# amankhullar/MMBiDAF

Hardware: NVIDIA B200
Metric: mmbidaf_train_videos_per_s (higher is better)
Workload: dtype bf16 tcgen05 BiDAF + tf32 library GEMMs, fp32 accumulate / soft-max / LSTM

## Files before the change

mmbidaf_b200/csrc/decoder_fused.cu:

```cuda
#include <cooperative_groups.h>
#include <stdlib.h>
#include <type_traits>
#include "common.cuh"
#include "tc_common.cuh"

namespace cg = cooperative_groups;

namespace mmb {
namespace {

constexpr int NT = 512;
constexpr int NW = NT / 32;
constexpr int MAXC = 8;
constexpr int SCR = 2048;
__host__ __device__ constexpr int split4(int n, int parts) { return ((n + parts - 1) / parts + 3) & ~3; }

__device__ __forceinline__ float rcp_ftz(float x) {
  float y;
  asm("rcp.approx.ftz.f32 %0, %1;" : "=f"(y) : "f"(x));
  return y;
}

__device__ __forceinline__ void bulk_reduce_add_f32(float* dst, uint32_t src_smem, uint32_t bytes) {
  asm volatile("cp.reduce.async.bulk.global.shared::cta.bulk_group.add.f32 [%0], [%1], %2;" ::"l"(dst), "r"(src_smem), "r"(bytes)
               : "memory");
}
__device__ __forceinline__ void bulk_commit() { asm volatile("cp.async.bulk.commit_group;" ::: "memory"); }
__device__ __forceinline__ void bulk_wait_all() { asm volatile("cp.async.bulk.wait_group 0;" ::: "memory"); }
__device__ __forceinline__ void red_add_f32_if(float* p, float v, bool on) {
  asm volatile(
      "{\n\t"
      ".reg .pred q;\n\t"
      "setp.ne.b32 q, %2, 0;\n\t"
      "@q red.global.add.f32 [%0], %1;\n\t"
      "}" ::"l"(p), "f"(v), "r"((int)on)
      : "memory");
}

__device__ long long* g_dec_trace = nullptr;
#define DEC_STAMP(i)                                                          \
  do {                                                                        \
    if (g_dec_trace && blockIdx.x == 0 && threadIdx.x == 0) g_dec_trace[i] = clock64(); \
  } while (0)

struct FusedArgs {
  const float *proj_a, *proj_i, *enc_a, *enc_i;
  const float *Wh4t, *bh4;
  const float *v1, *wc1, *v2, *wc2, *v1b, *v2b;
  const float *Wb13t;
  const float *vb1, *vb2, *vb1b, *vb2b;
  const float *Wcatt, *bcat;
  const float *out_wt, *out_b;
  const float *sent, *h, *cell, *cov;
  const uint8_t* mask;
  const long long* target;
  float *probs, *h_out, *cell_out, *att_cov, *cov_out;
  long long* argmax;
  float *nll, *cov_loss;
  float *hw, *alpha, *beta, *ctx12, *pb, *xcat, *gates;
  int B, Lt, D, H, E, M, chunk;
  int stage_off;
};

template <typename ColOf, typename Emit>
__device__ __forceinline__ void block_matvec_t(const float* __restrict__ Wt, const int ldn, const float* __restrict__ bias, const float* x,
                                               const int K, const int n_out, float* scratch, const int scratch_cap, bool quads,
                                               ColOf col_of, Emit emit) {
  const int tid = threadIdx.x;
  if (n_out <= 0) return;
  quads = quads && ((ldn | n_out) & 3) == 0 && (reinterpret_cast<uintptr_t>(Wt) & 15) == 0 && scratch_cap >= 2 * n_out;
  if (quads) {
    const int nq = n_out >> 2;
    const int S = max(1, min(min(NT / nq, scratch_cap / n_out), K));
    const int q = tid % nq, sl = tid / nq;
    float4 acc = make_float4(0.f, 0.f, 0.f, 0.f);
    if (sl < S) {
      const int per = (K + S - 1) / S, k0 = min(K, sl * per), k1 = min(K, k0 + per);
      const float4* w = reinterpret_cast<const float4*>(Wt + (size_t)k0 * ldn + col_of(4 * q));
      const size_t ld4 = (size_t)(ldn >> 2);
      for (int k = k0; k < k1; k += 16) {
        float4 wv[16];
#pragma unroll
        for (int u = 0; u < 16; ++u) wv[u] = k + u < k1 ? __ldcg(w + u * ld4) : make_float4(0.f, 0.f, 0.f, 0.f);
#pragma unroll
        for (int u = 0; u < 16; ++u) {
          const float xv = k + u < k1 ? x[k + u] : 0.f;
          acc.x = fmaf(wv[u].x, xv, acc.x); acc.y = fmaf(wv[u].y, xv, acc.y);
          acc.z = fmaf(wv[u].z, xv, acc.z); acc.w = fmaf(wv[u].w, xv, acc.w);
        }
        w += 16 * ld4;
      }
    }
    __syncthreads();
    if (sl < S) *reinterpret_cast<float4*>(scratch + sl * n_out + 4 * q) = acc;
    __syncthreads();
    if (tid < n_out) {
      float v = 0.f;
      for (int p = 0; p < S; ++p) v += scratch[p * n_out + tid];
      const int c = col_of(tid);
      emit(tid, v + (bias ? __ldg(bias + c) : 0.f));
    }
    return;
  }
  const int S = max(1, min(min(NT / n_out, scratch_cap / n_out), 32));
  const int i = tid % n_out, sl = tid / n_out;
  float acc = 0.f;
  if (sl < S) {
    const int per = (K + S - 1) / S, k0 = min(K, sl * per), k1 = min(K, k0 + per);
    const float* w = Wt + (size_t)k0 * ldn + col_of(i);
    float a0 = 0.f, a1 = 0.f, a2 = 0.f, a3 = 0.f;
    int k = k0;
    for (; k + 16 <= k1; k += 16) {
      float wv[16];
#pragma unroll
      for (int u = 0; u < 16; ++u) wv[u] = __ldcg(w + (size_t)u * ldn);
#pragma unroll
      for (int u = 0; u < 16; u += 4) {
        a0 = fmaf(wv[u], x[k + u], a0); a1 = fmaf(wv[u + 1], x[k + u + 1], a1);
        a2 = fmaf(wv[u + 2], x[k + u + 2], a2); a3 = fmaf(wv[u + 3], x[k + u + 3], a3);
      }
      w += (size_t)16 * ldn;
    }
    if (k + 8 <= k1) {
      float wv[8];
#pragma unroll
      for (int u = 0; u < 8; ++u) wv[u] = __ldcg(w + (size_t)u * ldn);
#pragma unroll
      for (int u = 0; u < 8; u += 4) {
        a0 = fmaf(wv[u], x[k + u], a0); a1 = fmaf(wv[u + 1], x[k + u + 1], a1);
        a2 = fmaf(wv[u + 2], x[k + u + 2], a2); a3 = fmaf(wv[u + 3], x[k + u + 3], a3);
      }
      w += (size_t)8 * ldn;
      k += 8;
    }
    for (; k < k1; ++k) {
      a0 = fmaf(__ldcg(w), x[k], a0);
      w += ldn;
    }
    acc = (a0 + a1) + (a2 + a3);
  }
  __syncthreads();
  if (sl < S && S > 1) scratch[sl * n_out + i] = acc;
  __syncthreads();
  if (tid < n_out) {
    float v = acc;
    for (int q = 1; q < S; ++q) v += scratch[q * n_out + tid];
    const int c = col_of(tid);
    emit(tid, v + (bias ? __ldg(bias + c) : 0.f));
  }
}

__device__ __forceinline__ float block_sum(float v, float* red) {
  const int lane = threadIdx.x & 31, warp = threadIdx.x >> 5;
  v = warp_sum(v);
  __syncthreads();
  if (lane == 0) red[warp] = v;
  __syncthreads();
  float r = lane < NW ? red[lane] : 0.f;
  return warp_sum(r);
}
__device__ __forceinline__ float block_max(float v, float* red) {
  const int lane = threadIdx.x & 31, warp = threadIdx.x >> 5;
  v = warp_max(v);
  __syncthreads();
  if (lane == 0) red[warp] = v;
  __syncthreads();
  float r = lane < NW ? red[lane] : -INFINITY;
  return warp_max(r);
}

struct GreedyArgs {
  const float *emb_text, *h0;
  int steps, T;
};

template <bool kGreedy>
__device__ __forceinline__ void dec_fused_body(const FusedArgs& a, const GreedyArgs& g) {
  cg::cluster_group cluster = cg::this_cluster();
  const int CL = (int)cluster.num_blocks(), R = (int)cluster.block_rank();
  const int b = blockIdx.x / CL;
  const int tid = threadIdx.x, lane = tid & 31, warp = tid >> 5;
  const int D = a.D, H = a.H, E = a.E, M = a.M, Lt = a.Lt, K = D + E + H;

  extern __shared__ __align__(16) float smem[];
  auto up4 = [](int v) { return (v + 3) & ~3; };
  float* s_hw = smem;
  float* s_x = s_hw + up4(4 * D);
  float* s_ctx = s_x + up4(K);
  float* s_pb = s_ctx + up4(2 * D);
  float* s_hn = s_pb + up4(2 * D);
  float* s_part = s_hn + up4(H);
  float* s_ex = s_part + up4(MAXC * (4 + 2 * D));
  float* s_g = s_ex + MAXC * 8;
  float* s_red = s_g + up4(4 * (split4(H, MAXC / 2) + 1));
  float* s_scr = s_red + 32;
  float* s_vec = s_scr + SCR;
  float* s_e = s_vec + up4(4 * D);
  float* s_cov = s_e + up4(2 * a.chunk);
  float* s_cpart = s_cov + up4(a.chunk);

  const int t0 = min(Lt, R * a.chunk), t1 = min(Lt, t0 + a.chunk), n = t1 - t0;
  const bool staged = a.stage_off != 0;
  float* const s_st0 = smem + a.stage_off + 4;
  float* const s_st1 = s_st0 + up4(a.chunk * D);
  const uint32_t bar_proj = tc::smem_u32(smem + a.stage_off), bar_enc = bar_proj + 8;
  const uint32_t stage_bytes = (uint32_t)(n * D) * 4u;
  if (staged && tid == 0) {
    tc::mbar_init(bar_proj, 1);
    tc::mbar_init(bar_enc, 1);
    tc::fence_barrier_init();
    if (n > 0) {
      tc::mbar_expect_tx(bar_proj, 2 * stage_bytes, 1);
      tc::tma_bulk_g2s(tc::smem_u32(s_st0), a.proj_a + ((size_t)b * Lt + t0) * D, stage_bytes, bar_proj, 1);
      tc::tma_bulk_g2s(tc::smem_u32(s_st1), a.proj_i + ((size_t)b * Lt + t0) * D, stage_bytes, bar_proj, 1);
    }
  }
  DEC_STAMP(0);
  const int S = kGreedy ? g.steps : 1;
  float cell_own = 0.f;
  int pick = 0;
  for (int s = 0; s < S; ++s) {
  const uint32_t parity = kGreedy ? (uint32_t)(s & 1) : 0u;
  if constexpr (!kGreedy) {
    for (int i = tid; i < n; i += NT) s_cov[i] = a.cov[(size_t)b * Lt + t0 + i];
    for (int i = tid; i < H; i += NT) s_x[D + E + i] = a.h[(size_t)b * H + i];
    for (int i = tid; i < E; i += NT) s_x[D + i] = a.sent[(size_t)b * E + i];
  } else {
    if (s == 0)
      for (int i = tid; i < n; i += NT) s_cov[i] = 0.f;
    for (int i = tid; i < H; i += NT) s_x[D + E + i] = s == 0 ? g.h0[(size_t)b * H + i] : s_hn[i];
    const float* row = g.emb_text + ((size_t)b * Lt + min(pick, Lt - 1)) * E;
    for (int i = tid; i < E; i += NT) s_x[D + i] = s == 0 ? 0.f : row[i];
  }
  if (!kGreedy || s == 0)
    for (int i = tid; i < D; i += NT) {
      s_vec[i] = a.v1[i];
      s_vec[D + i] = a.wc1[i];
      s_vec[2 * D + i] = a.v2[i];
      s_vec[3 * D + i] = a.wc2[i];
    }
  __syncthreads();

  DEC_STAMP(1);
  {
    const int per = (4 * D + CL - 1) / CL, o0 = R * per, o1 = min(4 * D, o0 + per);
    block_matvec_t(a.Wh4t, 4 * D, a.bh4, s_x + D + E, H, o1 - o0, s_scr, SCR, (o0 & 3) == 0, [&](int i) { return o0 + i; }, [&](int i, float v) {
      const int o = o0 + i;
      for (int r = 0; r < CL; ++r) cluster.map_shared_rank(s_hw, r)[o] = v;
      if constexpr (!kGreedy) a.hw[(size_t)b * 4 * D + o] = v;
    });
  }
  DEC_STAMP(2);
  cluster.sync();
  DEC_STAMP(3);

  {
    const float v1b = a.v1b[0], v2b = a.v2b[0];
    constexpr float K2 = 2.0f * 1.4426950408889634f;
    auto energies = [&](const float* __restrict__ pa0, const float* __restrict__ pi0, auto nj_tag, auto ru_tag) {
      constexpr int NJ = decltype(nj_tag)::value, RU = decltype(ru_tag)::value;
      float va[NJ], ha[NJ], wa[NJ], vi[NJ], hi[NJ], wi[NJ];
#pragma unroll
      for (int j = 0; j < NJ; ++j) {
        const int d = lane + 32 * j;
        const bool in = d < D;
        const int dd = in ? d : 0;
        va[j] = in ? s_vec[dd] : 0.f;
        wa[j] = in ? s_vec[D + dd] * K2 : 0.f;
        ha[j] = in ? s_hw[dd] * K2 : 0.f;
        vi[j] = in ? s_vec[2 * D + dd] : 0.f;
        wi[j] = in ? s_vec[3 * D + dd] * K2 : 0.f;
        hi[j] = in ? s_hw[D + dd] * K2 : 0.f;
      }
      const float* const covp = s_cov;
      for (int i = warp * RU; i < n; i += NW * RU) {
        float s[RU][2];
        float pav[RU][NJ], piv[RU][NJ], cvs[RU];
#pragma unroll
        for (int u = 0; u < RU; ++u) {
          s[u][0] = s[u][1] = 0.f;
          const int r = min(i + u, n - 1);
          const float* pa = pa0 + (size_t)r * D;
          const float* pi = pi0 + (size_t)r * D;
          cvs[u] = covp[r];
#pragma unroll
          for (int j = 0; j < NJ; ++j) {
            const int d = lane + 32 * j;
            pav[u][j] = d < D ? pa[d] : 0.f;
            piv[u][j] = d < D ? pi[d] : 0.f;
          }
        }
#pragma unroll
        for (int u = 0; u < RU; ++u) {
          const float cv = cvs[u];
#pragma unroll
          for (int j = 0; j < NJ; ++j) {
            const float x1 = fmaf(cv, wa[j], fmaf(pav[u][j], K2, ha[j]));
            const float x2 = fmaf(cv, wi[j], fmaf(piv[u][j], K2, hi[j]));
            const float r1 = rcp_ftz(1.0f + tc::fast_exp2(x1)), r2 = rcp_ftz(1.0f + tc::fast_exp2(x2));
            s[u][0] = fmaf(va[j], fmaf(-2.0f, r1, 1.0f), s[u][0]);
            s[u][1] = fmaf(vi[j], fmaf(-2.0f, r2, 1.0f), s[u][1]);
          }
        }
#pragma unroll
        for (int u = 0; u < RU; ++u) {
          const float x1 = warp_sum(s[u][0]), x2 = warp_sum(s[u][1]);
          if (lane == 0 && i + u < n) {
            s_e[i + u] = x1 + v1b;
            s_e[a.chunk + i + u] = x2 + v2b;
          }
        }
      }
    };
    const float* const gpa = a.proj_a + ((size_t)b * Lt + t0) * D;
    const float* const gpi = a.proj_i + ((size_t)b * Lt + t0) * D;
    using N7 = std::integral_constant<int, 7>;
    using N8 = std::integral_constant<int, 8>;
    using R2 = std::integral_constant<int, 2>;
    using R4 = std::integral_constant<int, 4>;
    const bool nj7 = D > 192 && D <= 224;
    if (staged) {
      if (n > 0) tc::mbar_wait(bar_proj, parity);
      if (nj7) energies(s_st0, s_st1, N7{}, R2{});
      else energies(s_st0, s_st1, N8{}, R2{});
    } else {
      if (nj7) energies(gpa, gpi, N7{}, R4{});
      else energies(gpa, gpi, N8{}, R4{});
    }
    __syncthreads();
    if (staged && tid == 0 && n > 0) {
      tc::fence_proxy_async();
      tc::mbar_expect_tx(bar_enc, 2 * stage_bytes, 1);
      tc::tma_bulk_g2s(tc::smem_u32(s_st0), a.enc_a + ((size_t)b * Lt + t0) * D, stage_bytes, bar_enc, 1);
      tc::tma_bulk_g2s(tc::smem_u32(s_st1), a.enc_i + ((size_t)b * Lt + t0) * D, stage_bytes, bar_enc, 1);
    }
    DEC_STAMP(4);
    float m1 = -INFINITY, m2 = -INFINITY;
    for (int i = tid; i < n; i += NT) {
      m1 = fmaxf(m1, s_e[i]);
      m2 = fmaxf(m2, s_e[a.chunk + i]);
    }
    m1 = block_max(m1, s_red);
    m2 = block_max(m2, s_red);
    float l1 = 0.f, l2 = 0.f;
    for (int i = tid; i < n; i += NT) {
      const float p1 = expf(s_e[i] - m1), p2 = expf(s_e[a.chunk + i] - m2);
      s_e[i] = p1;
      s_e[a.chunk + i] = p2;
      l1 += p1;
      l2 += p2;
    }
    l1 = block_sum(l1, s_red);
    l2 = block_sum(l2, s_red);
    __syncthreads();
    DEC_STAMP(5);
    if (staged && n > 0) tc::mbar_wait(bar_enc, parity);
    const float* ea = staged ? s_st0 : a.enc_a + ((size_t)b * Lt + t0) * D;
    const float* ei = staged ? s_st1 : a.enc_i + ((size_t)b * Lt + t0) * D;
    const bool vec4 = (D & 3) == 0;
    const int groups = vec4 ? NT / (D >> 2) : NT / D;
    if (vec4) {
      const int dv4 = D >> 2;
      const int g = tid / dv4, c4 = tid - g * dv4;
      if (g < groups) {
        float4 s1 = make_float4(0.f, 0.f, 0.f, 0.f), s2 = s1;
#pragma unroll 8
        for (int i = g; i < n; i += groups) {
          const float w1 = s_e[i], w2 = s_e[a.chunk + i];
          const float4 x1 = *reinterpret_cast<const float4*>(ea + (size_t)i * D + c4 * 4);
          const float4 x2 = *reinterpret_cast<const float4*>(ei + (size_t)i * D + c4 * 4);
          s1.x = fmaf(w1, x1.x, s1.x); s1.y = fmaf(w1, x1.y, s1.y); s1.z = fmaf(w1, x1.z, s1.z); s1.w = fmaf(w1, x1.w, s1.w);
          s2.x = fmaf(w2, x2.x, s2.x); s2.y = fmaf(w2, x2.y, s2.y); s2.z = fmaf(w2, x2.z, s2.z); s2.w = fmaf(w2, x2.w, s2.w);
        }
        *reinterpret_cast<float4*>(s_cpart + (g * 2 + 0) * D + c4 * 4) = s1;
        *reinterpret_cast<float4*>(s_cpart + (g * 2 + 1) * D + c4 * 4) = s2;
      }
    } else {
      const int g = tid / D, d = tid - g * D;
      if (g < groups) {
        float s1 = 0.f, s2 = 0.f;
        for (int i = g; i < n; i += groups) {
          s1 = fmaf(s_e[i], ea[(size_t)i * D + d], s1);
          s2 = fmaf(s_e[a.chunk + i], ei[(size_t)i * D + d], s2);
        }
        s_cpart[(g * 2 + 0) * D + d] = s1;
        s_cpart[(g * 2 + 1) * D + d] = s2;
      }
    }
    __syncthreads();
    if constexpr (kGreedy) {
      if (staged && tid == 0 && n > 0 && s + 1 < S) {
        tc::fence_proxy_async();
        tc::mbar_expect_tx(bar_proj, 2 * stage_bytes, 1);
        tc::tma_bulk_g2s(tc::smem_u32(s_st0), a.proj_a + ((size_t)b * Lt + t0) * D, stage_bytes, bar_proj, 1);
        tc::tma_bulk_g2s(tc::smem_u32(s_st1), a.proj_i + ((size_t)b * Lt + t0) * D, stage_bytes, bar_proj, 1);
      }
    }
    for (int d = tid; d < 2 * D; d += NT) {
      const int k = d / D, dd = d - k * D;
      float s = 0.f;
      for (int g = 0; g < groups; ++g) s += s_cpart[(g * 2 + k) * D + dd];
      for (int r = 0; r < CL; ++r) cluster.map_shared_rank(s_part, r)[R * (4 + 2 * D) + 4 + d] = s;
    }
    if (tid < CL) {
      float* dst = cluster.map_shared_rank(s_part, tid) + R * (4 + 2 * D);
      dst[0] = m1; dst[1] = l1; dst[2] = m2; dst[3] = l2;
    }
  }
  DEC_STAMP(6);
  cluster.sync();
  DEC_STAMP(7);

  float scale_own[2];
  {
    float* s_w = s_scr;
    if (tid < 2) {
      const int k = tid;
      float m = -INFINITY;
      for (int r = 0; r < CL; ++r)
        if (min(Lt, r * a.chunk) < Lt) m = fmaxf(m, s_part[r * (4 + 2 * D) + 2 * k]);
      float l = 0.f, w[MAXC];
#pragma unroll
      for (int r = 0; r < MAXC; ++r) {
        w[r] = (r < CL && min(Lt, r * a.chunk) < Lt) ? expf(s_part[r * (4 + 2 * D) + 2 * k] - m) : 0.f;
        l = fmaf(w[r], r < CL ? s_part[r * (4 + 2 * D) + 2 * k + 1] : 0.f, l);
      }
      const float inv = 1.f / l;
#pragma unroll
      for (int r = 0; r < MAXC; ++r) s_w[k * MAXC + r] = w[r] * inv;
    }
    __syncthreads();
    scale_own[0] = s_w[R];
    scale_own[1] = s_w[MAXC + R];
    for (int i = tid; i < 2 * D; i += NT) {
      const int k = i / D;
      float sum = 0.f;
      for (int r = 0; r < CL; ++r) sum = fmaf(s_w[k * MAXC + r], s_part[r * (4 + 2 * D) + 4 + i], sum);
      s_ctx[i] = sum;
      if (!kGreedy && R == 0) a.ctx12[((size_t)k * a.B + b) * D + (i - k * D)] = sum;
    }
  }
  __syncthreads();
  DEC_STAMP(8);

  {
    const int per = (2 * D + CL - 1) / CL, o0 = R * per, o1 = min(2 * D, o0 + per);
    for (int k = 0; k < 2; ++k) {
      const int lo = max(o0, k * D), hi = min(o1, (k + 1) * D);
      block_matvec_t(a.Wb13t + (size_t)k * D * D, D, nullptr, s_ctx + k * D, D, hi - lo, s_scr, SCR, ((lo - k * D) & 3) == 0,
                     [&](int i) { return lo - k * D + i; },
                     [&](int i, float v) {
                       const int o = lo + i;
                       for (int r = 0; r < CL; ++r) cluster.map_shared_rank(s_pb, r)[o] = v;
                       if constexpr (!kGreedy) a.pb[((size_t)k * a.B + b) * D + (o - k * D)] = v;
                     });
    }
  }
  DEC_STAMP(9);
  cluster.sync();
  DEC_STAMP(10);
  float beta1, beta2;
  {
    float eb1 = 0.f, eb2 = 0.f;
    for (int d = tid; d < D; d += NT) {
      eb1 = fmaf(a.vb1[d], tanh_fast(s_pb[d] + s_hw[2 * D + d]), eb1);
      eb2 = fmaf(a.vb2[d], tanh_fast(s_pb[D + d] + s_hw[3 * D + d]), eb2);
    }
    eb1 = block_sum(eb1, s_red) + a.vb1b[0];
    eb2 = block_sum(eb2, s_red) + a.vb2b[0];
    const float mb = fmaxf(eb1, eb2);
    const float x1 = expf(eb1 - mb), x2 = expf(eb2 - mb);
    beta1 = x1 / (x1 + x2);
    beta2 = x2 / (x1 + x2);
    for (int d = tid; d < D; d += NT) s_x[d] = s_ctx[d] * beta1 + s_ctx[D + d] * beta2;
    float closs = 0.f;
    for (int i = tid; i < n; i += NT) {
      const int t = t0 + i;
      const float a1 = s_e[i] * scale_own[0], a2 = s_e[a.chunk + i] * scale_own[1];
      if constexpr (!kGreedy) {
        a.alpha[((size_t)b * 2 + 0) * Lt + t] = a1;
        a.alpha[((size_t)b * 2 + 1) * Lt + t] = a2;
      }
      const float att = a1 * beta1 + a2 * beta2;
      if constexpr (kGreedy) {
        const float cnew = s_cov[i] + att;
        s_cov[i] = cnew;
        closs += fminf(att, cnew);
      } else {
        const float cnew = a.cov[(size_t)b * Lt + t] + att;
        a.att_cov[(size_t)b * Lt + t] = att;
        a.cov_out[(size_t)b * Lt + t] = cnew;
        closs += fminf(att, cnew);
      }
    }
    closs = block_sum(closs, s_red);
    if (tid == 0) cluster.map_shared_rank(s_ex, 0)[R * 8 + 0] = closs;
    if (!kGreedy && R == 0 && tid == 0) {
      a.beta[b * 2 + 0] = beta1;
      a.beta[b * 2 + 1] = beta2;
    }
  }
  __syncthreads();
  if (!kGreedy && R == 0)
    for (int i = tid; i < K; i += NT) a.xcat[(size_t)b * K + i] = s_x[i];

  DEC_STAMP(11);
  {
    const int per = split4(H, CL), j0 = R * per, j1 = min(H, j0 + per), nj = max(0, j1 - j0);
    block_matvec_t(a.Wcatt, 4 * H, a.bcat, s_x, K, 4 * nj, s_scr, SCR, ((H | nj) & 3) == 0, [&](int i) { return (i / nj) * H + j0 + (i % nj); },
                   [&](int i, float v) { s_g[(i / nj) * (per + 1) + (i % nj)] = v; });
    __syncthreads();
    if (tid < nj) {
      const int j = j0 + tid;
      const float gi = gate_act(s_g[tid], 1.f), gf = gate_act(s_g[(per + 1) + tid], 1.f), gg = tanh_fast(s_g[2 * (per + 1) + tid]),
                  go = gate_act(s_g[3 * (per + 1) + tid], 1.f);
      const float c = fmaf(gf, kGreedy ? cell_own : a.cell[(size_t)b * H + j], gi * gg);
      const float hn = go * tanh_fast(c);
      if constexpr (kGreedy) {
        cell_own = c;
      } else {
        a.cell_out[(size_t)b * H + j] = c;
        a.h_out[(size_t)b * H + j] = hn;
        float* gs = a.gates + (size_t)b * 4 * H;
        gs[j] = gi; gs[H + j] = gf; gs[2 * H + j] = gg; gs[3 * H + j] = go;
      }
      for (int r = 0; r < CL; ++r) cluster.map_shared_rank(s_hn, r)[j] = hn;
    }
  }
  DEC_STAMP(12);
  cluster.sync();
  DEC_STAMP(13);
  const size_t prow = kGreedy ? (size_t)b * S + s : (size_t)b;
  const int lrow = kGreedy ? s * 2 * a.B + b : b;
  if (R == 0 && tid == 0 && a.cov_loss) {
    float cs = 0.f;
    for (int r = 0; r < CL; ++r) cs += s_ex[r * 8 + 0];
    a.cov_loss[lrow] = cs;
  }

  {
    const int per = (M + CL - 1) / CL, m0 = min(M, R * per), m1 = min(M, m0 + per);
    float* const lg = s_cpart;
    block_matvec_t(a.out_wt, M, a.out_b, s_hn, H, m1 - m0, s_scr, SCR, (m0 & 3) == 0, [&](int i) { return m0 + i; }, [&](int i, float v) { lg[i] = v; });
    __syncthreads();
    for (int m = m0 + tid; m < m1; m += NT)
      if (!a.mask[(size_t)b * M + m]) lg[m - m0] = kNegFill;
    __syncthreads();
    float mx = -INFINITY;
    for (int m = m0 + tid; m < m1; m += NT) mx = fmaxf(mx, lg[m - m0]);
    mx = block_max(mx, s_red);
    float sum = 0.f;
    for (int m = m0 + tid; m < m1; m += NT) sum += expf(lg[m - m0] - mx);
    sum = block_sum(sum, s_red);
    if (tid < CL) {
      float* dst = cluster.map_shared_rank(s_ex, tid) + R * 8;
      dst[1] = mx;
      dst[2] = sum;
    }
    DEC_STAMP(14);
    cluster.sync();
    DEC_STAMP(15);
    float gmx = -INFINITY;
    for (int r = 0; r < CL; ++r)
      if (min(M, r * per) < M) gmx = fmaxf(gmx, s_ex[r * 8 + 1]);
    float gsum = 0.f;
    for (int r = 0; r < CL; ++r)
      if (min(M, r * per) < M) gsum = fmaf(s_ex[r * 8 + 2], expf(s_ex[r * 8 + 1] - gmx), gsum);
    const float inv = 1.f / gsum;
    float best = -INFINITY;
    int best_i = M;
    const int tg = a.target ? (int)a.target[kGreedy ? b * g.T + s : b] : -1;
    for (int m = m0 + tid; m < m1; m += NT) {
      const float p = expf(lg[m - m0] - gmx) * inv;
      a.probs[prow * M + m] = p;
      if (p > best) { best = p; best_i = m; }
      if (m == tg && a.nll) a.nll[lrow] = -logf(p + 1e-12f);
    }
    if (kGreedy || a.argmax) {
      const float bbest = block_max(best, s_red);
      int cand = best == bbest ? best_i : M;
#pragma unroll
      for (int o = 16; o > 0; o >>= 1) cand = min(cand, __shfl_xor_sync(0xffffffffu, cand, o));
      __shared__ int redi[NW];
      __syncthreads();
      if (lane == 0) redi[warp] = cand;
      __syncthreads();
      if (tid == 0) {
        int r = M;
        for (int w = 0; w < NW; ++w) r = min(r, redi[w]);
        for (int q = 0; q < (kGreedy ? CL : 1); ++q) {
          float* dst = cluster.map_shared_rank(s_ex, q) + R * 8;
          dst[3] = bbest;
          dst[4] = __int_as_float(r);
        }
      }
      cluster.sync();
      if (kGreedy || (R == 0 && tid == 0)) {
        float gb = -INFINITY;
        int gi = M;
        for (int r = 0; r < CL; ++r) {
          if (min(M, r * per) >= M) continue;
          const float pb_ = s_ex[r * 8 + 3];
          const int ib = __float_as_int(s_ex[r * 8 + 4]);
          if (pb_ > gb || (pb_ == gb && ib < gi)) { gb = pb_; gi = ib; }
        }
        if constexpr (kGreedy) {
          if (R == 0 && tid == 0) a.argmax[prow] = gi;
          pick = gi;
        } else {
          a.argmax[b] = gi;
        }
      }
    }
  }
  }
  DEC_STAMP(16);
  DEC_STAMP(17);
}

__global__ void __launch_bounds__(NT) dec_step_fused_kernel(const FusedArgs a) { dec_fused_body<false>(a, GreedyArgs{}); }

__global__ void __launch_bounds__(NT) dec_greedy_fused_kernel(const FusedArgs a, const GreedyArgs g) { dec_fused_body<true>(a, g); }

}

struct HeadArgs {
  const float *probs, *d_probs;
  const long long* target;
  const float *g_nll, *g_cov;
  const float* out_w;
  const float *gates, *cell_in, *cell_out;
  const float *d_h_out, *d_cell_out;
  const float* Wcat_ctx;
  const float *d_att_cov, *d_cov_out;
  const float *alpha, *beta, *ctx12, *pb, *hw;
  const float *vb1, *vb2;
  const float *att, *cov_out;
  const float* Wb13;
  float* d_logits;
  float* d_gates;
  float *d_cell, *datt, *dcov_tot, *d_pre_b, *d_ctx12;
  float *vec_acc, *scal_acc;
  int B, Lt, D, H, M, ldd, ldg, chunk;
  int sweeps;
  const float *proj_a, *proj_i, *enc_a, *enc_i, *cov;
  const float *v1, *wc1, *v2, *wc2;
  float *d_proj_a, *d_proj_i, *d_cov;
  const float* Wh_stack;
  float* d_h;
  int stage_off;
};

__global__ void __launch_bounds__(NT) dec_bwd_head_kernel(const HeadArgs a) {
  cg::cluster_group cluster = cg::this_cluster();
  const int CL = (int)cluster.num_blocks(), R = (int)cluster.block_rank();
  const int b = blockIdx.x / CL;
  const int tid = threadIdx.x;
  const int D = a.D, H = a.H, M = a.M, Lt = a.Lt;

  extern __shared__ __align__(16) float smem[];
  auto up4 = [](int v) { return (v + 3) & ~3; };
  float* s_dl = smem;
  const int per_m = (M + CL - 1) / CL;
  float* s_dhp = s_dl + up4(per_m);
  float* s_dg = s_dhp + up4(MAXC * H);
  float* s_dctx = s_dg + up4(4 * H);
  float* s_dpre = s_dctx + up4(D);
  float* s_ex = s_dpre + up4(2 * D);
  float* s_red = s_ex + MAXC * 4;
  float* s_scr = s_red + 32;
  const int mv_cap = a.sweeps ? (a.stage_off != 0 ? NW / 2 : NW) * 3 * D : NT;
  float* const mv_scr = a.sweeps ? s_scr + NT + up4(2 * D) + up4(2 * a.chunk) + up4(4 * a.chunk) + up4(6 * D) : s_scr;
  const bool mv_quads = a.sweeps != 0;

  const int t0 = min(Lt, R * a.chunk), t1 = min(Lt, t0 + a.chunk), n = t1 - t0;
  const bool staged = a.stage_off != 0;
  float* const s_st0 = smem + a.stage_off + 4;
  float* const s_st1 = s_st0 + up4(a.chunk * D);
  const uint32_t bar_enc = tc::smem_u32(smem + a.stage_off), bar_proj = bar_enc + 8;
  const uint32_t stage_bytes = (uint32_t)(n * D) * 4u;
  if (staged && tid == 0) {
    tc::mbar_init(bar_enc, 1);
    tc::mbar_init(bar_proj, 1);
    tc::fence_barrier_init();
    if (n > 0) {
      tc::mbar_expect_tx(bar_enc, 2 * stage_bytes, 1);
      tc::tma_bulk_g2s(tc::smem_u32(s_st0), a.enc_a + ((size_t)b * Lt + t0) * D, stage_bytes, bar_enc, 1);
      tc::tma_bulk_g2s(tc::smem_u32(s_st1), a.enc_i + ((size_t)b * Lt + t0) * D, stage_bytes, bar_enc, 1);
    }
  }
  DEC_STAMP(18);
  const int m0 = min(M, R * per_m), m1 = min(M, m0 + per_m);
  const int tg = a.target ? (int)a.target[b] : -1;
  const float dp_t = a.target ? -a.g_nll[b] / (a.probs[(size_t)b * M + tg] + 1e-12f) : 0.f;
  if (a.d_probs) {
    float dot = 0.f;
    for (int m = m0 + tid; m < m1; m += NT) dot = fmaf(a.probs[(size_t)b * M + m], a.d_probs[(size_t)b * M + m], dot);
    dot = block_sum(dot, s_red);
    if (tid < CL) cluster.map_shared_rank(s_ex, tid)[R * 4 + 0] = dot;
    cluster.sync();
  }
  {
    float dot = 0.f;
    if (a.d_probs)
      for (int r = 0; r < CL; ++r) dot += s_ex[r * 4 + 0];
    if (a.target) dot = fmaf(a.probs[(size_t)b * M + tg], dp_t, dot);
    for (int m = m0 + tid; m < m1; m += NT) {
      const float dp = (a.d_probs ? a.d_probs[(size_t)b * M + m] : 0.f) + (m == tg ? dp_t : 0.f);
      const float v = a.probs[(size_t)b * M + m] * (dp - dot);
      s_dl[m - m0] = v;
      a.d_logits[(size_t)b * a.ldd + m] = v;
    }
    if (R == 0)
      for (int m = M + tid; m < a.ldd; m += NT) a.d_logits[(size_t)b * a.ldd + m] = 0.f;
  }
  __syncthreads();
  DEC_STAMP(19);
  block_matvec_t(a.out_w + (size_t)m0 * H, H, nullptr, s_dl, m1 - m0, H, mv_scr, mv_cap, mv_quads, [](int i) { return i; }, [&](int i, float v) {
    for (int r = 0; r < CL; ++r) cluster.map_shared_rank(s_dhp, r)[R * H + i] = v;
  });
  if (m1 - m0 <= 0 && tid < H)
    for (int r = 0; r < CL; ++r) cluster.map_shared_rank(s_dhp, r)[R * H + tid] = 0.f;
  cluster.sync();
  DEC_STAMP(20);
  if (tid < H) {
    const int j = tid;
    float dh = 0.f;
    for (int r = 0; r < CL; ++r) dh += s_dhp[r * H + j];
    if (a.d_h_out) dh += a.d_h_out[(size_t)b * H + j];
    const float* g = a.gates + (size_t)b * 4 * H;
    const float gi = g[j], gf = g[H + j], gg = g[2 * H + j], go = g[3 * H + j];
    const float tc = tanh_fast(a.cell_out[(size_t)b * H + j]);
    const float dc = fmaf(dh * go, 1.f - tc * tc, a.d_cell_out ? a.d_cell_out[(size_t)b * H + j] : 0.f);
    const float di = dc * gg * gi * (1.f - gi), df = dc * a.cell_in[(size_t)b * H + j] * gf * (1.f - gf);
    const float dg = dc * gi * (1.f - gg * gg), dO = dh * tc * go * (1.f - go);
    s_dg[j] = di; s_dg[H + j] = df; s_dg[2 * H + j] = dg; s_dg[3 * H + j] = dO;
    if (R == 0) {
      float* o = a.d_gates + (size_t)b * a.ldg;
      o[j] = di; o[H + j] = df; o[2 * H + j] = dg; o[3 * H + j] = dO;
      a.d_cell[(size_t)b * H + j] = dc * gf;
    }
  }
  __syncthreads();
  DEC_STAMP(21);
  {
    const int per = split4(D, CL), d0 = min(D, R * per), d1 = min(D, d0 + per);
    block_matvec_t(a.Wcat_ctx, D, nullptr, s_dg, 4 * H, d1 - d0, mv_scr, mv_cap, mv_quads, [&](int i) { return d0 + i; }, [&](int i, float v) {
      for (int r = 0; r < CL; ++r) cluster.map_shared_rank(s_dctx, r)[d0 + i] = v;
    });
  }
  cluster.sync();
  DEC_STAMP(22);
  const float beta1 = a.beta[b * 2 + 0], beta2 = a.beta[b * 2 + 1];
  {
    float db1 = 0.f, db2 = 0.f;
    if (R == 0)
      for (int d = tid; d < D; d += NT) {
        db1 = fmaf(a.ctx12[(size_t)b * D + d], s_dctx[d], db1);
        db2 = fmaf(a.ctx12[((size_t)a.B + b) * D + d], s_dctx[d], db2);
      }
    const float gc = a.g_cov ? a.g_cov[b] : 0.f;
    const int t0 = min(Lt, R * a.chunk), t1 = min(Lt, t0 + a.chunk);
    for (int t = t0 + tid; t < t1; t += NT) {
      float dcv = a.d_cov_out ? a.d_cov_out[(size_t)b * Lt + t] : 0.f;
      float g = a.d_att_cov ? a.d_att_cov[(size_t)b * Lt + t] : 0.f;
      if (a.g_cov) {
        const float av = a.att[(size_t)b * Lt + t], cv = a.cov_out[(size_t)b * Lt + t];
        const float tie = av == cv ? 0.5f * gc : 0.f;
        g += av < cv ? gc : tie;
        dcv += cv < av ? gc : tie;
      }
      a.dcov_tot[(size_t)b * Lt + t] = dcv;
      g += dcv;
      a.datt[(size_t)b * Lt + t] = g;
      db1 = fmaf(a.alpha[((size_t)b * 2 + 0) * Lt + t], g, db1);
      db2 = fmaf(a.alpha[((size_t)b * 2 + 1) * Lt + t], g, db2);
    }
    db1 = block_sum(db1, s_red);
    db2 = block_sum(db2, s_red);
    if (tid < CL) {
      float* dst = cluster.map_shared_rank(s_ex, tid) + R * 4;
      dst[1] = db1;
      dst[2] = db2;
    }
  }
  cluster.sync();
  {
    float db1 = 0.f, db2 = 0.f;
    for (int r = 0; r < CL; ++r) {
      db1 += s_ex[r * 4 + 1];
      db2 += s_ex[r * 4 + 2];
    }
    const float mix = beta1 * db1 + beta2 * db2;
    const float deb1 = beta1 * (db1 - mix), deb2 = beta2 * (db2 - mix);
    for (int d = tid; d < D; d += NT) {
      const float t1 = tanh_fast(a.pb[(size_t)b * D + d] + a.hw[(size_t)b * 4 * D + 2 * D + d]);
      const float t2 = tanh_fast(a.pb[((size_t)a.B + b) * D + d] + a.hw[(size_t)b * 4 * D + 3 * D + d]);
      const float p1 = deb1 * a.vb1[d] * (1.f - t1 * t1), p2 = deb2 * a.vb2[d] * (1.f - t2 * t2);
      s_dpre[d] = p1;
      s_dpre[D + d] = p2;
      if (R == 0) {
        a.d_pre_b[(size_t)b * D + d] = p1;
        a.d_pre_b[((size_t)a.B + b) * D + d] = p2;
        a.vec_acc[((size_t)b * 6 + 4) * D + d] += deb1 * t1;
        a.vec_acc[((size_t)b * 6 + 5) * D + d] += deb2 * t2;
      }
    }
    if (R == 0 && tid == 0) {
      a.scal_acc[b * 4 + 2] += deb1;
      a.scal_acc[b * 4 + 3] += deb2;
    }
  }
  __syncthreads();
  DEC_STAMP(23);
  float* s_dc = s_scr + NT;
  {
    const int per = (2 * D + CL - 1) / CL, o0 = min(2 * D, R * per), o1 = min(2 * D, o0 + per);
    for (int k = 0; k < 2; ++k) {
      const int lo = max(o0, k * D), hi = min(o1, (k + 1) * D);
      const float bk = k == 0 ? beta1 : beta2;
      block_matvec_t(a.Wb13 + (size_t)k * D * D, D, nullptr, s_dpre + k * D, D, hi - lo, mv_scr, mv_cap, mv_quads && ((lo - k * D) & 3) == 0,
                     [&](int i) { return lo - k * D + i; },
                     [&](int i, float v) {
                       const int dd = lo - k * D + i;
                       const float x = fmaf(bk, s_dctx[dd], v);
                       a.d_ctx12[((size_t)k * a.B + b) * D + dd] = x;
                       if (a.sweeps)
                         for (int r = 0; r < CL; ++r) cluster.map_shared_rank(s_dc, r)[k * D + dd] = x;
                     });
    }
  }
  cluster.sync();
  if (!a.sweeps) return;

  const int lane = tid & 31, warp = tid >> 5;
  auto up4s = [](int v) { return (v + 3) & ~3; };
  float* s_da = s_dc + up4s(2 * D);
  float* s_rowc = s_da + up4s(2 * a.chunk);
  float* s_vec = s_rowc + up4s(4 * a.chunk);
  const int PW = staged ? NW / 2 : NW;
  float* s_part = s_vec + up4s(6 * D);
  float* s_row = s_part + up4s(PW * 3 * D);
  float* s_colp = s_row + up4s(a.chunk);
  float* s_in = s_colp + up4s(CL * 6 * D);
  using N7 = std::integral_constant<int, 7>;
  using N8 = std::integral_constant<int, 8>;
  const bool nj7 = D > 192 && D <= 224;
  DEC_STAMP(24);
  for (int i = tid; i < D; i += NT) {
    s_vec[i] = a.v1[i];
    s_vec[D + i] = a.wc1[i];
    s_vec[2 * D + i] = a.hw[(size_t)b * 4 * D + i];
    s_vec[3 * D + i] = a.v2[i];
    s_vec[4 * D + i] = a.wc2[i];
    s_vec[5 * D + i] = a.hw[(size_t)b * 4 * D + D + i];
  }
  for (int i = tid; i < n; i += NT) {
    s_row[i] = a.dcov_tot[(size_t)b * Lt + t0 + i];
    s_rowc[i] = a.alpha[((size_t)b * 2 + 0) * Lt + t0 + i];
    s_rowc[a.chunk + i] = a.alpha[((size_t)b * 2 + 1) * Lt + t0 + i];
    s_rowc[2 * a.chunk + i] = a.datt[(size_t)b * Lt + t0 + i];
    s_rowc[3 * a.chunk + i] = a.cov[(size_t)b * Lt + t0 + i];
  }
  __syncthreads();
  float s1 = 0.f, s2 = 0.f;
  auto sweep7 = [&](const float* __restrict__ ea0, const float* __restrict__ ei0, auto nj_tag) {
    constexpr int NJ = decltype(nj_tag)::value;
    float dca[NJ], dci[NJ];
#pragma unroll
    for (int j = 0; j < NJ; ++j) {
      const int d = lane + 32 * j;
      dca[j] = d < D ? s_dc[d] : 0.f;
      dci[j] = d < D ? s_dc[D + d] : 0.f;
    }
    for (int i = warp * 2; i < n; i += NW * 2) {
      float d1[2] = {0.f, 0.f}, d2[2] = {0.f, 0.f};
      float eav[2][NJ], eiv[2][NJ];
#pragma unroll
      for (int u = 0; u < 2; ++u) {
        const float* ea = ea0 + (size_t)min(i + u, n - 1) * D;
        const float* ei = ei0 + (size_t)min(i + u, n - 1) * D;
#pragma unroll
        for (int j = 0; j < NJ; ++j) {
          const int d = lane + 32 * j;
          eav[u][j] = d < D ? ea[d] : 0.f;
          eiv[u][j] = d < D ? ei[d] : 0.f;
        }
      }
#pragma unroll
      for (int u = 0; u < 2; ++u)
#pragma unroll
        for (int j = 0; j < NJ; ++j) {
          d1[u] = fmaf(dca[j], eav[u][j], d1[u]);
          d2[u] = fmaf(dci[j], eiv[u][j], d2[u]);
        }
#pragma unroll
      for (int u = 0; u < 2; ++u) {
        const float x1 = warp_sum(d1[u]), x2 = warp_sum(d2[u]);
        if (lane == 0 && i + u < n) {
          const float g = s_rowc[2 * a.chunk + i + u];
          const float da1 = x1 + beta1 * g, da2 = x2 + beta2 * g;
          s_da[i + u] = da1;
          s_da[a.chunk + i + u] = da2;
          s1 = fmaf(s_rowc[i + u], da1, s1);
          s2 = fmaf(s_rowc[a.chunk + i + u], da2, s2);
        }
      }
    }
  };
  if (staged) {
    if (n > 0) tc::mbar_wait(bar_enc, 0);
    if (nj7) sweep7(s_st0, s_st1, N7{}); else sweep7(s_st0, s_st1, N8{});
  } else {
    const float* const gea = a.enc_a + ((size_t)b * Lt + t0) * D;
    const float* const gei = a.enc_i + ((size_t)b * Lt + t0) * D;
    if (nj7) sweep7(gea, gei, N7{}); else sweep7(gea, gei, N8{});
  }
  {
    s1 = block_sum(s1, s_red);
    if (staged && tid == 0 && n > 0) {
      tc::fence_proxy_async();
      tc::mbar_expect_tx(bar_proj, 2 * stage_bytes, 1);
      tc::tma_bulk_g2s(tc::smem_u32(s_st0), a.proj_a + ((size_t)b * Lt + t0) * D, stage_bytes, bar_proj, 1);
      tc::tma_bulk_g2s(tc::smem_u32(s_st1), a.proj_i + ((size_t)b * Lt + t0) * D, stage_bytes, bar_proj, 1);
    }
    s2 = block_sum(s2, s_red);
    if (tid < CL) {
      float* dst = cluster.map_shared_rank(s_ex, tid) + R * 4;
      dst[0] = s1;
      dst[1] = s2;
    }
  }
  cluster.sync();
  float stot0 = 0.f, stot1 = 0.f;
  for (int r = 0; r < CL; ++r) {
    stot0 += s_ex[r * 4 + 0];
    stot1 += s_ex[r * 4 + 1];
  }
  DEC_STAMP(25);
  for (int i = tid; i < n; i += NT) {
    s_da[i] = s_rowc[i] * (s_da[i] - stot0);
    s_da[a.chunk + i] = s_rowc[a.chunk + i] * (s_da[a.chunk + i] - stot1);
  }
  __syncthreads();
  constexpr float K2 = 2.0f * 1.4426950408889634f;
  float se_m0 = 0.f, se_m1 = 0.f;
  auto sweep8 = [&](const int m, float* proj, auto nj_tag, auto staged_tag) {
    constexpr int NJ = decltype(nj_tag)::value;
    constexpr bool STAGED = decltype(staged_tag)::value;
    float* dproj = (m == 0 ? a.d_proj_a : a.d_proj_i) + ((size_t)b * Lt + t0) * D;
    float vvr[NJ], wcr[NJ], hwk[NJ];
    float c_dz[NJ], c_cov[NJ], c_v[NJ];
#pragma unroll
    for (int j = 0; j < NJ; ++j) {
      const int d = lane + 32 * j;
      const float* vv = s_vec + 3 * m * D;
      vvr[j] = d < D ? vv[d] : 0.f;
      wcr[j] = d < D ? vv[D + d] : 0.f;
      hwk[j] = d < D ? vv[2 * D + d] * K2 : 0.f;
      c_dz[j] = c_cov[j] = c_v[j] = 0.f;
    }
    float se = 0.f;
    for (int i0 = warp * 2; i0 < n; i0 += NW * 2) {
      float cvs[2], dets[2], pv[2][NJ];
#pragma unroll
      for (int u = 0; u < 2; ++u) {
        const int i = min(i0 + u, n - 1);
        cvs[u] = s_rowc[3 * a.chunk + i];
        dets[u] = i0 + u < n ? s_da[m * a.chunk + i] : 0.f;
#pragma unroll
        for (int j = 0; j < NJ; ++j) {
          const int d = lane + 32 * j;
          pv[u][j] = d < D ? proj[(size_t)i * D + d] : 0.f;
        }
      }
#pragma unroll
      for (int u = 0; u < 2; ++u) {
        const int i = i0 + u;
        const bool valid = i < n;
        const float cv = cvs[u], det = dets[u], cvk = cv * K2;
        float row = 0.f;
#pragma unroll
        for (int j = 0; j < NJ; ++j) {
          const int d = lane + 32 * j;
          const float tz = fmaf(-2.0f, rcp_ftz(1.0f + tc::fast_exp2(fmaf(cvk, wcr[j], fmaf(pv[u][j], K2, hwk[j])))), 1.0f);
          const float dz = det * vvr[j] * (1.f - tz * tz);
          if (STAGED) {
            if (valid && d < D) proj[(size_t)i * D + d] = dz;
          } else {
            red_add_f32_if(dproj + (size_t)i * D + d, dz, valid && d < D);
          }
          c_dz[j] += dz;
          c_cov[j] = fmaf(dz, cv, c_cov[j]);
          c_v[j] = fmaf(det, tz, c_v[j]);
          row = fmaf(dz, wcr[j], row);
        }
        row = warp_sum(row);
        if (lane == 0 && valid) {
          s_row[i] += row;
          se += det;
        }
      }
    }
    if (STAGED) tc::fence_proxy_async();
    se = block_sum(se, s_red);
    if (m == 0) se_m0 = se; else se_m1 = se;
    if (STAGED && tid == 0 && n > 0) {
      bulk_reduce_add_f32(dproj, tc::smem_u32(proj), stage_bytes);
      bulk_commit();
    }
    float xacc[2] = {0.f, 0.f};
    for (int w0 = 0; w0 < NW; w0 += PW) {
      if (warp >= w0 && warp < w0 + PW) {
#pragma unroll
        for (int j = 0; j < NJ; ++j) {
          const int d = lane + 32 * j;
          if (d < D) {
            s_part[((warp - w0) * 3 + 0) * D + d] = c_dz[j];
            s_part[((warp - w0) * 3 + 1) * D + d] = c_cov[j];
            s_part[((warp - w0) * 3 + 2) * D + d] = c_v[j];
          }
        }
      }
      __syncthreads();
#pragma unroll
      for (int q = 0; q < 2; ++q) {
        const int i = tid + q * NT;
        if (i < 3 * D)
          for (int w = 0; w < PW; ++w) xacc[q] += s_part[w * 3 * D + i];
      }
      __syncthreads();
    }
#pragma unroll
    for (int q = 0; q < 2; ++q) {
      const int i = tid + q * NT;
      if (i < 3 * D)
        for (int r = 0; r < CL; ++r) cluster.map_shared_rank(s_colp, r)[(R * 2 + m) * 3 * D + i] = xacc[q];
    }
  };
  if (staged && n > 0) tc::mbar_wait(bar_proj, 0);
  for (int m = 0; m < 2; ++m) {
    if (staged) {
      float* const sp = m == 0 ? s_st0 : s_st1;
      if (nj7) sweep8(m, sp, N7{}, std::true_type{}); else sweep8(m, sp, N8{}, std::true_type{});
    } else {
      float* const gp = const_cast<float*>(m == 0 ? a.proj_a : a.proj_i) + ((size_t)b * Lt + t0) * D;
      if (nj7) sweep8(m, gp, N7{}, std::false_type{}); else sweep8(m, gp, N8{}, std::false_type{});
    }
  }
  for (int i = tid; i < n; i += NT) a.d_cov[(size_t)b * Lt + t0 + i] = s_row[i];
  if (tid < CL) {
    float* dst = cluster.map_shared_rank(s_ex, tid) + R * 4;
    dst[2] = se_m0;
    dst[3] = se_m1;
  }
  cluster.sync();
  DEC_STAMP(26);
  for (int i = tid; i < 2 * D; i += NT) {
    const int m = i / D, d = i - m * D;
    float x = 0.f, y = 0.f, z = 0.f;
    for (int r = 0; r < CL; ++r) {
      const float* q = s_colp + (r * 2 + m) * 3 * D;
      x += q[d];
      y += q[D + d];
      z += q[2 * D + d];
    }
    s_in[4 * H + m * D + d] = x;
    s_in[4 * H + (2 + m) * D + d] = s_dpre[m * D + d];
    if (R == 0) {
      float* o = a.d_gates + (size_t)b * a.ldg + 4 * H;
      o[m * D + d] = x;
      o[(2 + m) * D + d] = s_dpre[m * D + d];
      a.vec_acc[((size_t)b * 6 + m) * D + d] += y;
      a.vec_acc[((size_t)b * 6 + 2 + m) * D + d] += z;
    }
  }
  for (int i = tid; i < 4 * H; i += NT) s_in[i] = s_dg[i];
  if (R == 0 && tid < 2) {
    float sv = 0.f;
    for (int r = 0; r < CL; ++r) sv += s_ex[r * 4 + 2 + tid];
    a.scal_acc[b * 4 + tid] += sv;
  }
  __syncthreads();
  {
    const int per = split4(H, CL), j0 = min(H, R * per), j1 = min(H, j0 + per);
    block_matvec_t(a.Wh_stack, H, nullptr, s_in, 4 * H + 4 * D, j1 - j0, mv_scr, mv_cap, mv_quads, [&](int i) { return j0 + i; },
                   [&](int i, float v) { a.d_h[(size_t)b * H + j0 + i] = v; });
  }
  if (staged && tid == 0) bulk_wait_all();
  DEC_STAMP(27);
}

static size_t g_head_smem_set = 0;

static size_t head_smem_bytes(int D, int H, int M, int CL, int chunk = 0, bool sweeps = false, int PW = NW) {
  auto up4 = [](size_t v) { return (v + 3) & ~(size_t)3; };
  const size_t per_m = (M + CL - 1) / CL;
  size_t floats = up4(per_m) + up4((size_t)MAXC * H) + up4(4 * H) + up4(D) + up4(2 * D) + MAXC * 4 + 32 + NT;
  if (sweeps)
    floats += up4(2 * D) + up4(2 * (size_t)chunk) + up4(4 * (size_t)chunk) + up4(6 * D) + up4((size_t)PW * 3 * D) + up4(chunk) + up4((size_t)CL * 6 * D) +
              up4(4 * H + 4 * D);
  return floats * sizeof(float) + 64;
}

static size_t fused_smem_bytes(int Lt, int D, int H, int E, int M, int CL, int* chunk_out) {
  const int chunk = (Lt + CL - 1) / CL;
  const int K = D + E + H;
  const int groups = (D & 3) == 0 ? NT / (D >> 2) : NT / D;
  const int per_m = (M + CL - 1) / CL;
  int cpart = groups * 2 * D;
  if (cpart < per_m) cpart = per_m;
  auto up4 = [](size_t v) { return (v + 3) & ~(size_t)3; };
  const size_t floats = up4(4 * D) + up4(K) + 2 * up4(2 * D) + up4(H) + up4((size_t)MAXC * (4 + 2 * D)) + MAXC * 8 +
                        up4(4 * (split4(H, MAXC / 2) + 1)) + 32 + SCR + up4(4 * D) + up4(2 * (size_t)chunk) + up4(chunk) + up4(cpart);
  if (chunk_out) *chunk_out = chunk;
  return floats * sizeof(float) + 64;
}

static int launch_fused(FusedArgs a, const GreedyArgs* g, const char* who, mmb_stream_t stream) {
  const int B = a.B, Lt = a.Lt, D = a.D, H = a.H, E = a.E, M = a.M;
  MMB_REQUIRE(B > 0 && Lt > 0 && D > 0 && H > 0 && E >= 0 && M > 0, MMB_ERR_INVALID,
              "%s: B=%d Lt=%d D=%d H=%d E=%d M=%d", who, B, Lt, D, H, E, M);
  MMB_REQUIRE(D <= 256, MMB_ERR_UNSUPPORTED, "%s: D=%d > 256", who, D);
  const int CL = (long long)B * 4 * 2 <= 160 ? 8 : 4;
  size_t smem = fused_smem_bytes(Lt, D, H, E, M, CL, &a.chunk);
  MMB_REQUIRE(smem <= 200 * 1024, MMB_ERR_UNSUPPORTED, "%s: %zu B of shared memory (Lt=%d)", who, smem, Lt);
  {
    static const char* stage_env = getenv("MMB_DEC_STAGE");
    const size_t base_floats = (smem + 15) / 16 * 4;
    const size_t stage_floats = 4 + 2 * (((size_t)a.chunk * D + 3) & ~(size_t)3);
    const bool aligned = ((reinterpret_cast<uintptr_t>(a.proj_a) | reinterpret_cast<uintptr_t>(a.proj_i) |
                           reinterpret_cast<uintptr_t>(a.enc_a) | reinterpret_cast<uintptr_t>(a.enc_i)) & 15) == 0;
    if ((D & 3) == 0 && aligned && (base_floats + stage_floats) * 4 <= 227 * 1024 && !(stage_env && atoi(stage_env) == 0)) {
      a.stage_off = (int)base_floats;
      smem = (base_floats + stage_floats) * 4;
    }
  }
  static size_t smem_set[2] = {0, 0};
  if (smem > smem_set[g != nullptr]) {
    if (g) MMB_CUDA(cudaFuncSetAttribute(dec_greedy_fused_kernel, cudaFuncAttributeMaxDynamicSharedMemorySize, (int)smem));
    else MMB_CUDA(cudaFuncSetAttribute(dec_step_fused_kernel, cudaFuncAttributeMaxDynamicSharedMemorySize, (int)smem));
    smem_set[g != nullptr] = smem;
  }
  static const char* trace_env = getenv("MMB_DEC_TRACE");
  static bool trace_set = false;
  if (trace_env && !trace_set) {
    long long* ptr = reinterpret_cast<long long*>(strtoull(trace_env, nullptr, 0));
    MMB_CUDA(cudaMemcpyToSymbol(g_dec_trace, &ptr, sizeof(ptr)));
    trace_set = true;
  }
  cudaLaunchConfig_t cfg{};
  cfg.gridDim = dim3((unsigned)(B * CL));
  cfg.blockDim = dim3(NT);
  cfg.dynamicSmemBytes = smem;
  cfg.stream = static_cast<cudaStream_t>(stream);
  cudaLaunchAttribute attr[1];
  attr[0].id = cudaLaunchAttributeClusterDimension;
  attr[0].val.clusterDim.x = (unsigned)CL;
  attr[0].val.clusterDim.y = 1;
  attr[0].val.clusterDim.z = 1;
  cfg.attrs = attr;
  cfg.numAttrs = 1;
  if (g) {
    MMB_CUDA(cudaLaunchKernelEx(&cfg, dec_greedy_fused_kernel, a, *g));
    return check_launch("dec_greedy_fused_kernel");
  }
  MMB_CUDA(cudaLaunchKernelEx(&cfg, dec_step_fused_kernel, a));
  return check_launch("dec_step_fused_kernel");
}

}

extern "C" int mmb_decoder_step_fused_fwd(const float* proj_a, const float* proj_i, const float* enc_a, const float* enc_i,
                                          const float* Wh4t, const float* bh4, const float* v1, const float* wc1, const float* v2,
                                          const float* wc2, const float* v1b, const float* v2b, const float* Wb13t, const float* vb1,
                                          const float* vb2, const float* vb1b, const float* vb2b, const float* Wcatt,
                                          const float* bcat, const float* out_wt, const float* out_b, const float* sent,
                                          const float* h, const float* cell, const float* cov, const uint8_t* mask,
                                          const long long* target, float* probs, float* h_out, float* cell_out, float* att_cov,
                                          float* cov_out, long long* argmax, float* nll, float* cov_loss, float* hw, float* alpha,
                                          float* beta, float* ctx12, float* pb, float* xcat, float* gates, int B, int Lt, int D,
                                          int H, int E, int M, mmb_stream_t stream) {
  using namespace mmb;
  MMB_REQUIRE(proj_a && proj_i && enc_a && enc_i && Wh4t && bh4 && v1 && wc1 && v2 && wc2 && v1b && v2b && Wb13t && vb1 && vb2 &&
                  vb1b && vb2b && Wcatt && bcat && out_wt && out_b && sent && h && cell && cov && mask && probs && h_out &&
                  cell_out && att_cov && cov_out && hw && alpha && beta && ctx12 && pb && xcat && gates,
              MMB_ERR_INVALID, "mmb_decoder_step_fused_fwd: null pointer");
  FusedArgs a{proj_a, proj_i, enc_a, enc_i, Wh4t, bh4, v1, wc1, v2, wc2, v1b, v2b, Wb13t, vb1, vb2, vb1b, vb2b, Wcatt, bcat, out_wt, out_b,
              sent, h, cell, cov, mask, target, probs, h_out, cell_out, att_cov, cov_out, argmax, nll, cov_loss, hw, alpha, beta,
              ctx12, pb, xcat, gates, B, Lt, D, H, E, M, 0, 0};
  return launch_fused(a, nullptr, "mmb_decoder_step_fused_fwd", stream);
}

extern "C" int mmb_decoder_greedy_fused(const float* proj_a, const float* proj_i, const float* enc_a, const float* enc_i,
                                        const float* Wh4t, const float* bh4, const float* v1, const float* wc1, const float* v2,
                                        const float* wc2, const float* v1b, const float* v2b, const float* Wb13t, const float* vb1,
                                        const float* vb2, const float* vb1b, const float* vb2b, const float* Wcatt, const float* bcat,
                                        const float* out_wt, const float* out_b, const float* emb_text, const float* h0,
                                        const uint8_t* mask, const long long* target, float* probs, long long* argmax,
                                        float* loss_terms, int B, int Lt, int D, int H, int E, int M, int S, int T,
                                        mmb_stream_t stream) {
  using namespace mmb;
  MMB_REQUIRE(proj_a && proj_i && enc_a && enc_i && Wh4t && bh4 && v1 && wc1 && v2 && wc2 && v1b && v2b && Wb13t && vb1 && vb2 &&
                  vb1b && vb2b && Wcatt && bcat && out_wt && out_b && emb_text && h0 && mask && probs && argmax,
              MMB_ERR_INVALID, "mmb_decoder_greedy_fused: null pointer");
  MMB_REQUIRE(S > 0 && (!target || (loss_terms && T >= S)), MMB_ERR_INVALID, "mmb_decoder_greedy_fused: S=%d T=%d, target %s, loss_terms %s",
              S, T, target ? "set" : "null", loss_terms ? "set" : "null");
  FusedArgs a{proj_a, proj_i, enc_a, enc_i, Wh4t, bh4, v1, wc1, v2, wc2, v1b, v2b, Wb13t, vb1, vb2, vb1b, vb2b, Wcatt, bcat, out_wt, out_b,
              nullptr, nullptr, nullptr, nullptr, mask, target, probs, nullptr, nullptr, nullptr, nullptr, argmax,
              target ? loss_terms : nullptr, target ? loss_terms + B : nullptr, nullptr, nullptr, nullptr, nullptr, nullptr, nullptr,
              nullptr, B, Lt, D, H, E, M, 0, 0};
  const GreedyArgs g{emb_text, h0, S, target ? T : 0};
  return launch_fused(a, &g, "mmb_decoder_greedy_fused", stream);
}

extern "C" int mmb_decoder_bwd_head(const float* probs, const float* d_probs, const long long* target, const float* g_nll,
                                    const float* g_cov, const float* out_w, const float* gates, const float* cell_in,
                                    const float* cell_out, const float* d_h_out, const float* d_cell_out, const float* Wcat_ctx,
                                    const float* d_att_cov, const float* d_cov_out, const float* alpha, const float* beta,
                                    const float* ctx12, const float* pb, const float* hw, const float* vb1, const float* vb2,
                                    const float* att, const float* cov_out, const float* Wb13, float* d_logits, int ldd, float* d_gates,
                                    int ldg, float* d_cell, float* datt, float* dcov_tot, float* d_pre_b, float* d_ctx12, float* vec_acc,
                                    float* scal_acc, int B, int Lt, int D, int H, int M, mmb_stream_t stream) {
  using namespace mmb;
  MMB_REQUIRE(probs && out_w && gates && cell_in && cell_out && Wcat_ctx && alpha && beta && ctx12 && pb && hw && vb1 && vb2 && Wb13 &&
                  d_logits && d_gates && d_cell && datt && dcov_tot && d_pre_b && d_ctx12 && vec_acc && scal_acc,
              MMB_ERR_INVALID, "mmb_decoder_bwd_head: null pointer");
  MMB_REQUIRE((!target || g_nll) && (!g_cov || (att && cov_out)), MMB_ERR_INVALID, "mmb_decoder_bwd_head: loss-term pointers");
  MMB_REQUIRE(B > 0 && Lt > 0 && D > 0 && H > 0 && M > 0 && ldd >= M && ldg >= 4 * H && H <= NT, MMB_ERR_INVALID,
              "mmb_decoder_bwd_head: B=%d Lt=%d D=%d H=%d M=%d ldd=%d ldg=%d", B, Lt, D, H, M, ldd, ldg);
  const int CL = (long long)B * 4 * 2 <= 160 ? 8 : 4;
  HeadArgs a{probs, d_probs, target, g_nll, g_cov, out_w, gates, cell_in, cell_out, d_h_out, d_cell_out, Wcat_ctx, d_att_cov, d_cov_out,
             alpha, beta, ctx12, pb, hw, vb1, vb2, att, cov_out, Wb13, d_logits, d_gates, d_cell, datt, dcov_tot, d_pre_b, d_ctx12,
             vec_acc, scal_acc, B, Lt, D, H, M, ldd, ldg, (Lt + CL - 1) / CL,
             0, nullptr, nullptr, nullptr, nullptr, nullptr, nullptr, nullptr, nullptr, nullptr, nullptr, nullptr, nullptr, nullptr, nullptr, 0};
  const size_t smem = head_smem_bytes(D, H, M, CL);
  MMB_REQUIRE(smem <= 200 * 1024, MMB_ERR_UNSUPPORTED, "mmb_decoder_bwd_head: %zu B of shared memory", smem);
  if (smem > g_head_smem_set) {
    MMB_CUDA(cudaFuncSetAttribute(dec_bwd_head_kernel, cudaFuncAttributeMaxDynamicSharedMemorySize, (int)smem));
    g_head_smem_set = smem;
  }
  cudaLaunchConfig_t cfg{};
  cfg.gridDim = dim3((unsigned)(B * CL));
  cfg.blockDim = dim3(NT);
  cfg.dynamicSmemBytes = smem;
  cfg.stream = static_cast<cudaStream_t>(stream);
  cudaLaunchAttribute attr[1];
  attr[0].id = cudaLaunchAttributeClusterDimension;
  attr[0].val.clusterDim.x = (unsigned)CL;
  attr[0].val.clusterDim.y = 1;
  attr[0].val.clusterDim.z = 1;
  cfg.attrs = attr;
  cfg.numAttrs = 1;
  MMB_CUDA(cudaLaunchKernelEx(&cfg, dec_bwd_head_kernel, a));
  return check_launch("dec_bwd_head_kernel");
}

extern "C" int mmb_decoder_step_fused_bwd(const float* probs, const float* d_probs, const long long* target, const float* g_nll,
                                          const float* g_cov, const float* out_w, const float* gates, const float* cell_in,
                                          const float* cell_out, const float* d_h_out, const float* d_cell_out, const float* Wcat_ctx,
                                          const float* d_att_cov, const float* d_cov_out, const float* alpha, const float* beta,
                                          const float* ctx12, const float* pb, const float* hw, const float* vb1, const float* vb2,
                                          const float* att, const float* cov_out, const float* Wb13, float* d_logits, int ldd,
                                          float* d_gates, int ldg, float* d_cell, float* datt, float* dcov_tot, float* d_pre_b,
                                          float* d_ctx12, float* vec_acc, float* scal_acc, const float* proj_a, const float* proj_i,
                                          const float* enc_a, const float* enc_i, const float* coverage, const float* v1, const float* wc1,
                                          const float* v2, const float* wc2, float* d_proj_a, float* d_proj_i, float* d_cov,
                                          const float* Wh_stack, float* d_h, int B, int Lt, int D, int H, int M, mmb_stream_t stream) {
  using namespace mmb;
  MMB_REQUIRE(probs && out_w && gates && cell_in && cell_out && Wcat_ctx && alpha && beta && ctx12 && pb && hw && vb1 && vb2 && Wb13 &&
                  d_logits && d_gates && d_cell && datt && dcov_tot && d_pre_b && d_ctx12 && vec_acc && scal_acc && proj_a && proj_i &&
                  enc_a && enc_i && coverage && v1 && wc1 && v2 && wc2 && d_proj_a && d_proj_i && d_cov && Wh_stack && d_h,
              MMB_ERR_INVALID, "mmb_decoder_step_fused_bwd: null pointer");
  MMB_REQUIRE((!target || g_nll) && (!g_cov || (att && cov_out)), MMB_ERR_INVALID, "mmb_decoder_step_fused_bwd: loss-term pointers");
  MMB_REQUIRE(B > 0 && Lt > 0 && D > 0 && D <= 256 && H > 0 && M > 0 && ldd >= M && ldg >= 4 * H + 4 * D && H <= NT, MMB_ERR_INVALID,
              "mmb_decoder_step_fused_bwd: B=%d Lt=%d D=%d H=%d M=%d ldd=%d ldg=%d", B, Lt, D, H, M, ldd, ldg);
  const int CL = (long long)B * 4 * 2 <= 160 ? 8 : 4;
  const int chunk = (Lt + CL - 1) / CL;
  HeadArgs a{probs, d_probs, target, g_nll, g_cov, out_w, gates, cell_in, cell_out, d_h_out, d_cell_out, Wcat_ctx, d_att_cov, d_cov_out,
             alpha, beta, ctx12, pb, hw, vb1, vb2, att, cov_out, Wb13, d_logits, d_gates, d_cell, datt, dcov_tot, d_pre_b, d_ctx12,
             vec_acc, scal_acc, B, Lt, D, H, M, ldd, ldg, chunk,
             1, proj_a, proj_i, enc_a, enc_i, coverage, v1, wc1, v2, wc2, d_proj_a, d_proj_i, d_cov, Wh_stack, d_h, 0};
  size_t smem = head_smem_bytes(D, H, M, CL, chunk, true);
  MMB_REQUIRE(smem <= 200 * 1024, MMB_ERR_UNSUPPORTED, "mmb_decoder_step_fused_bwd: %zu B of shared memory (Lt=%d)", smem, Lt);
  {
    static const char* stage_env = getenv("MMB_DEC_STAGE");
    const size_t base_floats = (head_smem_bytes(D, H, M, CL, chunk, true, NW / 2) - 64) / 4;
    const size_t stage_floats = 4 + 2 * (((size_t)chunk * D + 3) & ~(size_t)3);
    const bool aligned = ((reinterpret_cast<uintptr_t>(proj_a) | reinterpret_cast<uintptr_t>(proj_i) | reinterpret_cast<uintptr_t>(enc_a) |
                           reinterpret_cast<uintptr_t>(enc_i) | reinterpret_cast<uintptr_t>(d_proj_a) |
                           reinterpret_cast<uintptr_t>(d_proj_i)) & 15) == 0;
    if ((D & 3) == 0 && aligned && (base_floats + stage_floats) * 4 + 64 <= 227 * 1024 && !(stage_env && atoi(stage_env) == 0)) {
      a.stage_off = (int)base_floats;
      smem = (base_floats + stage_floats) * 4 + 64;
    }
  }
  if (smem > g_head_smem_set) {
    MMB_CUDA(cudaFuncSetAttribute(dec_bwd_head_kernel, cudaFuncAttributeMaxDynamicSharedMemorySize, (int)smem));
    g_head_smem_set = smem;
  }
  cudaLaunchConfig_t cfg{};
  cfg.gridDim = dim3((unsigned)(B * CL));
  cfg.blockDim = dim3(NT);
  cfg.dynamicSmemBytes = smem;
  cfg.stream = static_cast<cudaStream_t>(stream);
  cudaLaunchAttribute attr[1];
  attr[0].id = cudaLaunchAttributeClusterDimension;
  attr[0].val.clusterDim.x = (unsigned)CL;
  attr[0].val.clusterDim.y = 1;
  attr[0].val.clusterDim.z = 1;
  cfg.attrs = attr;
  cfg.numAttrs = 1;
  MMB_CUDA(cudaLaunchKernelEx(&cfg, dec_bwd_head_kernel, a));
  return check_launch("dec_bwd_head_kernel (whole step)");
}
```

mmbidaf_b200/csrc/tc_common.cuh:

```cuda
#pragma once
#include <cuda_bf16.h>
#include "common.cuh"

namespace mmb {
namespace tc {

constexpr int DPAD = 208;
constexpr int CHUNKS = DPAD / 8;
constexpr int GROUP_BYTES = CHUNKS * 128;
constexpr int TMEM_COLS = 512;
constexpr float LOG2E = 1.4426950408889634f, LN2 = 0.6931471805599453f;

__device__ __forceinline__ uint32_t smem_u32(const void* p) { return static_cast<uint32_t>(__cvta_generic_to_shared(p)); }

__device__ __forceinline__ uint32_t elect_one() {
  uint32_t pred;
  asm volatile(
      "{\n\t"
      ".reg .pred p;\n\t"
      "elect.sync _|p, 0xffffffff;\n\t"
      "selp.u32 %0, 1, 0, p;\n\t"
      "}"
      : "=r"(pred));
  return pred;
}
__device__ __forceinline__ int uniform_warp_idx() { return __shfl_sync(0xffffffffu, (int)(threadIdx.x >> 5), 0); }

__device__ __forceinline__ void mbar_init(uint32_t bar, uint32_t count) {
  asm volatile("mbarrier.init.shared::cta.b64 [%0], %1;" ::"r"(bar), "r"(count) : "memory");
}
__device__ __forceinline__ void mbar_expect_tx(uint32_t bar, uint32_t bytes, uint32_t leader) {
  asm volatile(
      "{\n\t"
      ".reg .pred q;\n\t"
      "setp.ne.b32 q, %2, 0;\n\t"
      "@q mbarrier.arrive.expect_tx.shared::cta.b64 _, [%0], %1;\n\t"
      "}" ::"r"(bar), "r"(bytes), "r"(leader)
      : "memory");
}
__device__ __forceinline__ void mbar_wait(uint32_t bar, uint32_t parity) {
#pragma unroll 1
  for (uint32_t spin = 0; spin < (1u << 26); ++spin) {
    uint32_t done;
    asm volatile(
        "{\n\t"
        ".reg .pred p;\n\t"
        "mbarrier.try_wait.parity.shared::cta.b64 p, [%1], %2;\n\t"
        "selp.u32 %0, 1, 0, p;\n\t"
        "}"
        : "=r"(done)
        : "r"(bar), "r"(parity)
        : "memory");
    if (done) return;
  }
  __trap();
}
__device__ __forceinline__ void tma_bulk_g2s(uint32_t dst, const void* src, uint32_t bytes, uint32_t bar, uint32_t leader) {
  asm volatile(
      "{\n\t"
      ".reg .pred q;\n\t"
      "setp.ne.b32 q, %4, 0;\n\t"
      "@q cp.async.bulk.shared::cluster.global.mbarrier::complete_tx::bytes [%0], [%1], %2, [%3];\n\t"
      "}" ::"r"(dst), "l"(src), "r"(bytes), "r"(bar), "r"(leader)
      : "memory");
}
__device__ __forceinline__ void fence_proxy_async() { asm volatile("fence.proxy.async.shared::cta;" ::: "memory"); }
__device__ __forceinline__ long long globaltimer_ns() {
  long long t;
  asm volatile("mov.u64 %0, %%globaltimer;" : "=l"(t));
  return t;
}
__device__ __forceinline__ void fence_proxy_async_all() { asm volatile("fence.proxy.async;" ::: "memory"); }
__device__ __forceinline__ void signal_counter(int* counter) {
  __threadfence();
  asm volatile("red.release.gpu.global.add.s32 [%0], 1;" ::"l"(counter) : "memory");
}
__device__ __forceinline__ void wait_counter(const int* counter, int target) {
#pragma unroll 1
  for (uint32_t spin = 0; spin < (1u << 24); ++spin) {
    int v;
    asm volatile("ld.acquire.gpu.global.s32 %0, [%1];" : "=r"(v) : "l"(counter) : "memory");
    if (v >= target) return;
    __nanosleep(64);
  }
  __trap();
}
__device__ __forceinline__ void fence_barrier_init() { asm volatile("fence.mbarrier_init.release.cluster;" ::: "memory"); }
__device__ __forceinline__ void tc_fence_before() { asm volatile("tcgen05.fence::before_thread_sync;" ::: "memory"); }
__device__ __forceinline__ void tc_fence_after() { asm volatile("tcgen05.fence::after_thread_sync;" ::: "memory"); }

__device__ __forceinline__ void tmem_alloc(uint32_t dst_smem, uint32_t cols) {
  asm volatile("tcgen05.alloc.cta_group::1.sync.aligned.shared::cta.b32 [%0], %1;" ::"r"(dst_smem), "r"(cols) : "memory");
  asm volatile("tcgen05.relinquish_alloc_permit.cta_group::1.sync.aligned;" ::: "memory");
}
__device__ __forceinline__ void tmem_dealloc(uint32_t taddr, uint32_t cols) {
  asm volatile("tcgen05.dealloc.cta_group::1.sync.aligned.b32 %0, %1;" ::"r"(taddr), "r"(cols) : "memory");
}
__device__ __forceinline__ void umma_bf16(uint32_t d_tmem, uint64_t a_desc, uint64_t b_desc, uint32_t idesc, uint32_t acc,
                                          uint32_t leader) {
  asm volatile(
      "{\n\t"
      ".reg .pred p, q;\n\t"
      "setp.ne.b32 p, %4, 0;\n\t"
      "setp.ne.b32 q, %5, 0;\n\t"
      "@q tcgen05.mma.cta_group::1.kind::f16 [%0], %1, %2, %3, p;\n\t"
      "}" ::"r"(d_tmem), "l"(a_desc), "l"(b_desc), "r"(idesc), "r"(acc), "r"(leader)
      : "memory");
}
__device__ __forceinline__ void umma_bf16_lh(uint32_t d_tmem, uint32_t a_lo, uint32_t a_hi, uint32_t b_lo, uint32_t b_hi,
                                             uint32_t idesc, uint32_t acc, uint32_t leader) {
  asm volatile(
      "{\n\t"
      ".reg .pred p, q;\n\t"
      ".reg .b64 da, db;\n\t"
      "setp.ne.b32 p, %6, 0;\n\t"
      "setp.ne.b32 q, %7, 0;\n\t"
      "mov.b64 da, {%1, %2};\n\t"
      "mov.b64 db, {%3, %4};\n\t"
      "@q tcgen05.mma.cta_group::1.kind::f16 [%0], da, db, %5, p;\n\t"
      "}" ::"r"(d_tmem), "r"(a_lo), "r"(a_hi), "r"(b_lo), "r"(b_hi), "r"(idesc), "r"(acc), "r"(leader)
      : "memory");
}
__device__ __forceinline__ uint32_t desc_lo(uint32_t addr, uint32_t lbo_bytes) { return ((addr & 0x3FFFFu) >> 4) | ((lbo_bytes >> 4) << 16); }
constexpr uint32_t desc_hi(uint32_t sbo_bytes) { return (sbo_bytes >> 4) | (1u << 14); }
__device__ __forceinline__ void umma_commit(uint32_t bar, uint32_t leader) {
  asm volatile(
      "{\n\t"
      ".reg .pred q;\n\t"
      "setp.ne.b32 q, %1, 0;\n\t"
      "@q tcgen05.commit.cta_group::1.mbarrier::arrive::one.shared::cluster.b64 [%0];\n\t"
      "}" ::"r"(bar), "r"(leader)
      : "memory");
}
__device__ __forceinline__ void tmem_wait_ld() { asm volatile("tcgen05.wait::ld.sync.aligned;" ::: "memory"); }
__device__ __forceinline__ void tmem_wait_st() { asm volatile("tcgen05.wait::st.sync.aligned;" ::: "memory"); }

__device__ __forceinline__ void tmem_ld16(uint32_t taddr, float* v) {
  uint32_t r[16];
  asm volatile(
      "tcgen05.ld.sync.aligned.32x32b.x16.b32 {%0,%1,%2,%3,%4,%5,%6,%7,%8,%9,%10,%11,%12,%13,%14,%15}, [%16];"
      : "=r"(r[0]), "=r"(r[1]), "=r"(r[2]), "=r"(r[3]), "=r"(r[4]), "=r"(r[5]), "=r"(r[6]), "=r"(r[7]), "=r"(r[8]),
        "=r"(r[9]), "=r"(r[10]), "=r"(r[11]), "=r"(r[12]), "=r"(r[13]), "=r"(r[14]), "=r"(r[15])
      : "r"(taddr)
      : "memory");
  tmem_wait_ld();
#pragma unroll
  for (int i = 0; i < 16; ++i) v[i] = __uint_as_float(r[i]);
}
__device__ __forceinline__ void tmem_st16(uint32_t taddr, const float* v) {
  asm volatile(
      "tcgen05.st.sync.aligned.32x32b.x16.b32 [%0], {%1,%2,%3,%4,%5,%6,%7,%8,%9,%10,%11,%12,%13,%14,%15,%16};" ::"r"(taddr),
      "r"(__float_as_uint(v[0])), "r"(__float_as_uint(v[1])), "r"(__float_as_uint(v[2])), "r"(__float_as_uint(v[3])),
      "r"(__float_as_uint(v[4])), "r"(__float_as_uint(v[5])), "r"(__float_as_uint(v[6])), "r"(__float_as_uint(v[7])),
      "r"(__float_as_uint(v[8])), "r"(__float_as_uint(v[9])), "r"(__float_as_uint(v[10])), "r"(__float_as_uint(v[11])),
      "r"(__float_as_uint(v[12])), "r"(__float_as_uint(v[13])), "r"(__float_as_uint(v[14])), "r"(__float_as_uint(v[15]))
      : "memory");
}

__device__ __forceinline__ uint64_t smem_desc(uint32_t addr, uint32_t lbo_bytes, uint32_t sbo_bytes) {
  return (uint64_t)((addr & 0x3FFFFu) >> 4) | ((uint64_t)(lbo_bytes >> 4) << 16) | ((uint64_t)(sbo_bytes >> 4) << 32) |
         (1ull << 46);
}
constexpr uint32_t idesc_bf16(int n, int b_mn_major, int m = 128) {
  return (1u << 4) | (1u << 7) | (1u << 10) | ((uint32_t)b_mn_major << 16) | ((uint32_t)(n >> 3) << 17) | ((uint32_t)(m >> 4) << 24);
}

__device__ __forceinline__ float fast_exp2(float x) {
  float y;
  asm("ex2.approx.ftz.f32 %0, %1;" : "=f"(y) : "f"(x));
  return y;
}

inline int round_up(int v, int m) { return (v + m - 1) / m * m; }

constexpr int PACK_ROWS = 128;
struct BidafPacks {
  __nv_bfloat16 *cw, *cp;
  __nv_bfloat16 *qs, *qp;
  __nv_bfloat16* tp;
  unsigned long long *c_words, *q_words;
  int* ready;
  long long* trace;
  int LcP, LqP;
  size_t c_pack, q_pack, bytes;
};
inline BidafPacks bidaf_packs(void* workspace, int B, int Lc, int Lq, bool modality_dropout) {
  BidafPacks p;
  p.LcP = round_up(Lc, PACK_ROWS);
  p.LqP = round_up(Lq, PACK_ROWS);
  p.c_pack = (size_t)B * (p.LcP / 8) * GROUP_BYTES;
  p.q_pack = (size_t)B * (p.LqP / 8) * GROUP_BYTES;
  char* ws = static_cast<char*>(workspace);
  p.cw = reinterpret_cast<__nv_bfloat16*>(ws);
  p.cp = reinterpret_cast<__nv_bfloat16*>(ws + p.c_pack);
  p.qs = reinterpret_cast<__nv_bfloat16*>(ws + 2 * p.c_pack);
  p.tp = reinterpret_cast<__nv_bfloat16*>(ws + 2 * p.c_pack + p.q_pack);
  char* next = ws + 2 * p.c_pack + 2 * p.q_pack;
  p.qp = p.qs;
  if (modality_dropout) {
    p.qp = reinterpret_cast<__nv_bfloat16*>(next);
    next += p.q_pack;
  }
  p.c_words = reinterpret_cast<unsigned long long*>(next);
  p.q_words = p.c_words + (size_t)B * (p.LcP / 64) * 2;
  const size_t used = ((size_t)(next - ws) + 16 * (size_t)B * (p.LcP / 64 + p.LqP / 64) + 255) / 256 * 256;
  p.ready = reinterpret_cast<int*>(ws + used);
  const size_t used2 = used + ((size_t)(B + 1) * 4 + 255) / 256 * 256;
  p.trace = reinterpret_cast<long long*>(ws + used2);
  p.bytes = used2 + 4096;
  return p;
}

}
}
```

Baseline: 7543.

## Replace cluster.sync with st.async mbarrier exchanges and enable PDL in decoder kernels

Every cluster-wide barrier in the fused decoder and backward-head kernels is replaced with remote st.async stores that signal per-site transaction-count mbarriers. Each consumer now waits only for the bytes it needs instead of a full cluster rendezvous. Programmatic dependent launch (griddepcontrol) is also enabled so barrier init and the cluster arrive can overlap the tail of the previous kernel. The exact byte-count bookkeeping must match every writer. In particular, the removed zero-fill for an empty m-range in the head kernel could leave a barrier short of its expected bytes and hang.

```diff
diff --git a/mmbidaf_b200/csrc/decoder_fused.cu b/mmbidaf_b200/csrc/decoder_fused.cu
--- a/mmbidaf_b200/csrc/decoder_fused.cu
+++ b/mmbidaf_b200/csrc/decoder_fused.cu
@@ -1,10 +1,7 @@
-#include <cooperative_groups.h>
 #include <stdlib.h>
 #include <type_traits>
 #include "common.cuh"
 #include "tc_common.cuh"
-
-namespace cg = cooperative_groups;
 
 namespace mmb {
 namespace {
@@ -19,6 +16,10 @@
   float y;
   asm("rcp.approx.ftz.f32 %0, %1;" : "=f"(y) : "f"(x));
   return y;
+}
+
+__device__ __forceinline__ void put(float* buf, int i, float v, uint32_t bar, int rank) {
+  tc::st_async_f32(tc::mapa(tc::smem_u32(buf + i), (uint32_t)rank), v, tc::mapa(bar, (uint32_t)rank));
 }
 
 __device__ __forceinline__ void bulk_reduce_add_f32(float* dst, uint32_t src_smem, uint32_t bytes) {
@@ -176,11 +177,24 @@
 
 template <bool kGreedy>
 __device__ __forceinline__ void dec_fused_body(const FusedArgs& a, const GreedyArgs& g) {
-  cg::cluster_group cluster = cg::this_cluster();
-  const int CL = (int)cluster.num_blocks(), R = (int)cluster.block_rank();
+  const int CL = (int)tc::cluster_size(), R = (int)tc::cluster_rank();
   const int b = blockIdx.x / CL;
   const int tid = threadIdx.x, lane = tid & 31, warp = tid >> 5;
   const int D = a.D, H = a.H, E = a.E, M = a.M, Lt = a.Lt, K = D + E + H;
+
+  enum { X_HW, X_PART, X_PB, X_CLOSS, X_HN, X_STAT, X_ARG, NX };
+  __shared__ __align__(8) uint64_t xbar_mem[NX];
+  auto xbar = [&](int site) { return tc::smem_u32(xbar_mem + site); };
+  const bool has_closs = a.cov_loss != nullptr, has_arg = kGreedy || a.argmax != nullptr;
+  auto arm = [&]() {
+    tc::mbar_expect_tx(xbar(X_HW), 4u * (4 * D), 1);
+    tc::mbar_expect_tx(xbar(X_PART), 4u * (CL * (4 + 2 * D)), 1);
+    tc::mbar_expect_tx(xbar(X_PB), 4u * (2 * D), 1);
+    tc::mbar_expect_tx(xbar(X_HN), 4u * H, 1);
+    tc::mbar_expect_tx(xbar(X_STAT), 8u * CL, 1);
+    if (has_closs && R == 0) tc::mbar_expect_tx(xbar(X_CLOSS), 4u * CL, 1);
+    if (has_arg && (kGreedy || R == 0)) tc::mbar_expect_tx(xbar(X_ARG), 8u * CL, 1);
+  };
 
   extern __shared__ __align__(16) float smem[];
   auto up4 = [](int v) { return (v + 3) & ~3; };
@@ -205,15 +219,21 @@
   float* const s_st1 = s_st0 + up4(a.chunk * D);
   const uint32_t bar_proj = tc::smem_u32(smem + a.stage_off), bar_enc = bar_proj + 8;
   const uint32_t stage_bytes = (uint32_t)(n * D) * 4u;
-  if (staged && tid == 0) {
-    tc::mbar_init(bar_proj, 1);
-    tc::mbar_init(bar_enc, 1);
+  if (tid == 0) {
+    for (int x = 0; x < NX; ++x) tc::mbar_init(xbar(x), 1);
+    if (staged) {
+      tc::mbar_init(bar_proj, 1);
+      tc::mbar_init(bar_enc, 1);
+    }
     tc::fence_barrier_init();
-    if (n > 0) {
-      tc::mbar_expect_tx(bar_proj, 2 * stage_bytes, 1);
-      tc::tma_bulk_g2s(tc::smem_u32(s_st0), a.proj_a + ((size_t)b * Lt + t0) * D, stage_bytes, bar_proj, 1);
-      tc::tma_bulk_g2s(tc::smem_u32(s_st1), a.proj_i + ((size_t)b * Lt + t0) * D, stage_bytes, bar_proj, 1);
-    }
+  }
+  tc::cluster_arrive_relaxed();
+  tc::grid_dependency_wait();
+  tc::launch_dependents();
+  if (tid == 0 && staged && n > 0) {
+    tc::mbar_expect_tx(bar_proj, 2 * stage_bytes, 1);
+    tc::tma_bulk_g2s(tc::smem_u32(s_st0), a.proj_a + ((size_t)b * Lt + t0) * D, stage_bytes, bar_proj, 1);
+    tc::tma_bulk_g2s(tc::smem_u32(s_st1), a.proj_i + ((size_t)b * Lt + t0) * D, stage_bytes, bar_proj, 1);
   }
   DEC_STAMP(0);
   const int S = kGreedy ? g.steps : 1;
@@ -221,6 +241,7 @@
   int pick = 0;
   for (int s = 0; s < S; ++s) {
   const uint32_t parity = kGreedy ? (uint32_t)(s & 1) : 0u;
+  if (tid == 0) arm();
   if constexpr (!kGreedy) {
     for (int i = tid; i < n; i += NT) s_cov[i] = a.cov[(size_t)b * Lt + t0 + i];
     for (int i = tid; i < H; i += NT) s_x[D + E + i] = a.h[(size_t)b * H + i];
@@ -242,16 +263,17 @@
   __syncthreads();
 
   DEC_STAMP(1);
+  if (s == 0) tc::cluster_wait();
   {
     const int per = (4 * D + CL - 1) / CL, o0 = R * per, o1 = min(4 * D, o0 + per);
     block_matvec_t(a.Wh4t, 4 * D, a.bh4, s_x + D + E, H, o1 - o0, s_scr, SCR, (o0 & 3) == 0, [&](int i) { return o0 + i; }, [&](int i, float v) {
       const int o = o0 + i;
-      for (int r = 0; r < CL; ++r) cluster.map_shared_rank(s_hw, r)[o] = v;
+      for (int r = 0; r < CL; ++r) put(s_hw, o, v, xbar(X_HW), r);
       if constexpr (!kGreedy) a.hw[(size_t)b * 4 * D + o] = v;
     });
   }
   DEC_STAMP(2);
-  cluster.sync();
+  tc::mbar_wait(xbar(X_HW), parity);
   DEC_STAMP(3);
 
   {
@@ -400,15 +422,18 @@
       const int k = d / D, dd = d - k * D;
       float s = 0.f;
       for (int g = 0; g < groups; ++g) s += s_cpart[(g * 2 + k) * D + dd];
-      for (int r = 0; r < CL; ++r) cluster.map_shared_rank(s_part, r)[R * (4 + 2 * D) + 4 + d] = s;
+      for (int r = 0; r < CL; ++r) put(s_part, R * (4 + 2 * D) + 4 + d, s, xbar(X_PART), r);
     }
     if (tid < CL) {
-      float* dst = cluster.map_shared_rank(s_part, tid) + R * (4 + 2 * D);
-      dst[0] = m1; dst[1] = l1; dst[2] = m2; dst[3] = l2;
+      const int o = R * (4 + 2 * D);
+      put(s_part, o + 0, m1, xbar(X_PART), tid);
+      put(s_part, o + 1, l1, xbar(X_PART), tid);
+      put(s_part, o + 2, m2, xbar(X_PART), tid);
+      put(s_part, o + 3, l2, xbar(X_PART), tid);
     }
   }
   DEC_STAMP(6);
-  cluster.sync();
+  tc::mbar_wait(xbar(X_PART), parity);
   DEC_STAMP(7);
 
   float scale_own[2];
@@ -451,13 +476,13 @@
                      [&](int i) { return lo - k * D + i; },
                      [&](int i, float v) {
                        const int o = lo + i;
-                       for (int r = 0; r < CL; ++r) cluster.map_shared_rank(s_pb, r)[o] = v;
+                       for (int r = 0; r < CL; ++r) put(s_pb, o, v, xbar(X_PB), r);
                        if constexpr (!kGreedy) a.pb[((size_t)k * a.B + b) * D + (o - k * D)] = v;
                      });
     }
   }
   DEC_STAMP(9);
-  cluster.sync();
+  tc::mbar_wait(xbar(X_PB), parity);
   DEC_STAMP(10);
   float beta1, beta2;
   {
@@ -494,7 +519,7 @@
       }
     }
     closs = block_sum(closs, s_red);
-    if (tid == 0) cluster.map_shared_rank(s_ex, 0)[R * 8 + 0] = closs;
+    if (tid == 0 && has_closs) put(s_ex, R * 8 + 0, closs, xbar(X_CLOSS), 0);
     if (!kGreedy && R == 0 && tid == 0) {
       a.beta[b * 2 + 0] = beta1;
       a.beta[b * 2 + 1] = beta2;
@@ -524,15 +549,16 @@
         float* gs = a.gates + (size_t)b * 4 * H;
         gs[j] = gi; gs[H + j] = gf; gs[2 * H + j] = gg; gs[3 * H + j] = go;
       }
-      for (int r = 0; r < CL; ++r) cluster.map_shared_rank(s_hn, r)[j] = hn;
+      for (int r = 0; r < CL; ++r) put(s_hn, j, hn, xbar(X_HN), r);
     }
   }
   DEC_STAMP(12);
-  cluster.sync();
+  tc::mbar_wait(xbar(X_HN), parity);
   DEC_STAMP(13);
   const size_t prow = kGreedy ? (size_t)b * S + s : (size_t)b;
   const int lrow = kGreedy ? s * 2 * a.B + b : b;
-  if (R == 0 && tid == 0 && a.cov_loss) {
+  if (R == 0 && tid == 0 && has_closs) {
+    tc::mbar_wait(xbar(X_CLOSS), parity);
     float cs = 0.f;
     for (int r = 0; r < CL; ++r) cs += s_ex[r * 8 + 0];
     a.cov_loss[lrow] = cs;
@@ -553,12 +579,11 @@
     for (int m = m0 + tid; m < m1; m += NT) sum += expf(lg[m - m0] - mx);
     sum = block_sum(sum, s_red);
     if (tid < CL) {
-      float* dst = cluster.map_shared_rank(s_ex, tid) + R * 8;
-      dst[1] = mx;
-      dst[2] = sum;
+      put(s_ex, R * 8 + 1, mx, xbar(X_STAT), tid);
+      put(s_ex, R * 8 + 2, sum, xbar(X_STAT), tid);
     }
     DEC_STAMP(14);
-    cluster.sync();
+    tc::mbar_wait(xbar(X_STAT), parity);
     DEC_STAMP(15);
     float gmx = -INFINITY;
     for (int r = 0; r < CL; ++r)
@@ -589,13 +614,12 @@
         int r = M;
         for (int w = 0; w < NW; ++w) r = min(r, redi[w]);
         for (int q = 0; q < (kGreedy ? CL : 1); ++q) {
-          float* dst = cluster.map_shared_rank(s_ex, q) + R * 8;
-          dst[3] = bbest;
-          dst[4] = __int_as_float(r);
-        }
-      }
-      cluster.sync();
+          put(s_ex, R * 8 + 3, bbest, xbar(X_ARG), q);
+          put(s_ex, R * 8 + 4, __int_as_float(r), xbar(X_ARG), q);
+        }
+      }
       if (kGreedy || (R == 0 && tid == 0)) {
+        tc::mbar_wait(xbar(X_ARG), parity);
         float gb = -INFINITY;
         int gi = M;
         for (int r = 0; r < CL; ++r) {
@@ -652,11 +676,13 @@
 };
 
 __global__ void __launch_bounds__(NT) dec_bwd_head_kernel(const HeadArgs a) {
-  cg::cluster_group cluster = cg::this_cluster();
-  const int CL = (int)cluster.num_blocks(), R = (int)cluster.block_rank();
+  const int CL = (int)tc::cluster_size(), R = (int)tc::cluster_rank();
   const int b = blockIdx.x / CL;
   const int tid = threadIdx.x;
   const int D = a.D, H = a.H, M = a.M, Lt = a.Lt;
+  enum { X_DOT, X_DHP, X_DCTX, X_DB, X_DC, X_S7, X_COLP, NX };
+  __shared__ __align__(8) uint64_t xbar_mem[NX];
+  auto xbar = [&](int site) { return tc::smem_u32(xbar_mem + site); };
 
   extern __shared__ __align__(16) float smem[];
   auto up4 = [](int v) { return (v + 3) & ~3; };
@@ -667,7 +693,7 @@
   float* s_dctx = s_dg + up4(4 * H);
   float* s_dpre = s_dctx + up4(D);
   float* s_ex = s_dpre + up4(2 * D);
-  float* s_red = s_ex + MAXC * 4;
+  float* s_red = s_ex + MAXC * 8;
   float* s_scr = s_red + 32;
   const int mv_cap = a.sweeps ? (a.stage_off != 0 ? NW / 2 : NW) * 3 * D : NT;
   float* const mv_scr = a.sweeps ? s_scr + NT + up4(2 * D) + up4(2 * a.chunk) + up4(4 * a.chunk) + up4(6 * D) : s_scr;
@@ -679,15 +705,30 @@
   float* const s_st1 = s_st0 + up4(a.chunk * D);
   const uint32_t bar_enc = tc::smem_u32(smem + a.stage_off), bar_proj = bar_enc + 8;
   const uint32_t stage_bytes = (uint32_t)(n * D) * 4u;
-  if (staged && tid == 0) {
-    tc::mbar_init(bar_enc, 1);
-    tc::mbar_init(bar_proj, 1);
+  if (tid == 0) {
+    for (int x = 0; x < NX; ++x) tc::mbar_init(xbar(x), 1);
+    if (staged) {
+      tc::mbar_init(bar_enc, 1);
+      tc::mbar_init(bar_proj, 1);
+    }
     tc::fence_barrier_init();
-    if (n > 0) {
-      tc::mbar_expect_tx(bar_enc, 2 * stage_bytes, 1);
-      tc::tma_bulk_g2s(tc::smem_u32(s_st0), a.enc_a + ((size_t)b * Lt + t0) * D, stage_bytes, bar_enc, 1);
-      tc::tma_bulk_g2s(tc::smem_u32(s_st1), a.enc_i + ((size_t)b * Lt + t0) * D, stage_bytes, bar_enc, 1);
-    }
+    if (a.d_probs) tc::mbar_expect_tx(xbar(X_DOT), 4u * CL, 1);
+    tc::mbar_expect_tx(xbar(X_DHP), 4u * (CL * H), 1);
+    tc::mbar_expect_tx(xbar(X_DCTX), 4u * D, 1);
+    tc::mbar_expect_tx(xbar(X_DB), 8u * CL, 1);
+    if (a.sweeps) {
+      tc::mbar_expect_tx(xbar(X_DC), 4u * (2 * D), 1);
+      tc::mbar_expect_tx(xbar(X_S7), 8u * CL, 1);
+      tc::mbar_expect_tx(xbar(X_COLP), 4u * (CL * (2 * 3 * D + 2)), 1);
+    }
+  }
+  tc::cluster_arrive_relaxed();
+  tc::grid_dependency_wait();
+  tc::launch_dependents();
+  if (tid == 0 && staged && n > 0) {
+    tc::mbar_expect_tx(bar_enc, 2 * stage_bytes, 1);
+    tc::tma_bulk_g2s(tc::smem_u32(s_st0), a.enc_a + ((size_t)b * Lt + t0) * D, stage_bytes, bar_enc, 1);
+    tc::tma_bulk_g2s(tc::smem_u32(s_st1), a.enc_i + ((size_t)b * Lt + t0) * D, stage_bytes, bar_enc, 1);
   }
   DEC_STAMP(18);
   const int m0 = min(M, R * per_m), m1 = min(M, m0 + per_m);
@@ -697,13 +738,16 @@
     float dot = 0.f;
     for (int m = m0 + tid; m < m1; m += NT) dot = fmaf(a.probs[(size_t)b * M + m], a.d_probs[(size_t)b * M + m], dot);
     dot = block_sum(dot, s_red);
-    if (tid < CL) cluster.map_shared_rank(s_ex, tid)[R * 4 + 0] = dot;
-    cluster.sync();
+    tc::cluster_wait();
+    if (tid < CL) put(s_ex, R * 8 + 0, dot, xbar(X_DOT), tid);
+    tc::mbar_wait(xbar(X_DOT), 0);
+  } else {
+    tc::cluster_wait();
   }
   {
     float dot = 0.f;
     if (a.d_probs)
-      for (int r = 0; r < CL; ++r) dot += s_ex[r * 4 + 0];
+      for (int r = 0; r < CL; ++r) dot += s_ex[r * 8 + 0];
     if (a.target) dot = fmaf(a.probs[(size_t)b * M + tg], dp_t, dot);
     for (int m = m0 + tid; m < m1; m += NT) {
       const float dp = (a.d_probs ? a.d_probs[(size_t)b * M + m] : 0.f) + (m == tg ? dp_t : 0.f);
@@ -717,11 +761,9 @@
   __syncthreads();
   DEC_STAMP(19);
   block_matvec_t(a.out_w + (size_t)m0 * H, H, nullptr, s_dl, m1 - m0, H, mv_scr, mv_cap, mv_quads, [](int i) { return i; }, [&](int i, float v) {
-    for (int r = 0; r < CL; ++r) cluster.map_shared_rank(s_dhp, r)[R * H + i] = v;
+    for (int r = 0; r < CL; ++r) put(s_dhp, R * H + i, v, xbar(X_DHP), r);
   });
-  if (m1 - m0 <= 0 && tid < H)
-    for (int r = 0; r < CL; ++r) cluster.map_shared_rank(s_dhp, r)[R * H + tid] = 0.f;
-  cluster.sync();
+  tc::mbar_wait(xbar(X_DHP), 0);
   DEC_STAMP(20);
   if (tid < H) {
     const int j = tid;
@@ -746,10 +788,10 @@
   {
     const int per = split4(D, CL), d0 = min(D, R * per), d1 = min(D, d0 + per);
     block_matvec_t(a.Wcat_ctx, D, nullptr, s_dg, 4 * H, d1 - d0, mv_scr, mv_cap, mv_quads, [&](int i) { return d0 + i; }, [&](int i, float v) {
-      for (int r = 0; r < CL; ++r) cluster.map_shared_rank(s_dctx, r)[d0 + i] = v;
+      for (int r = 0; r < CL; ++r) put(s_dctx, d0 + i, v, xbar(X_DCTX), r);
     });
   }
-  cluster.sync();
+  tc::mbar_wait(xbar(X_DCTX), 0);
   DEC_STAMP(22);
   const float beta1 = a.beta[b * 2 + 0], beta2 = a.beta[b * 2 + 1];
   {
@@ -779,17 +821,16 @@
     db1 = block_sum(db1, s_red);
     db2 = block_sum(db2, s_red);
     if (tid < CL) {
-      float* dst = cluster.map_shared_rank(s_ex, tid) + R * 4;
-      dst[1] = db1;
-      dst[2] = db2;
-    }
-  }
-  cluster.sync();
+      put(s_ex, R * 8 + 1, db1, xbar(X_DB), tid);
+      put(s_ex, R * 8 + 2, db2, xbar(X_DB), tid);
+    }
+  }
+  tc::mbar_wait(xbar(X_DB), 0);
   {
     float db1 = 0.f, db2 = 0.f;
     for (int r = 0; r < CL; ++r) {
-      db1 += s_ex[r * 4 + 1];
-      db2 += s_ex[r * 4 + 2];
+      db1 += s_ex[r * 8 + 1];
+      db2 += s_ex[r * 8 + 2];
     }
     const float mix = beta1 * db1 + beta2 * db2;
     const float deb1 = beta1 * (db1 - mix), deb2 = beta2 * (db2 - mix);
@@ -826,11 +867,10 @@
                        const float x = fmaf(bk, s_dctx[dd], v);
                        a.d_ctx12[((size_t)k * a.B + b) * D + dd] = x;
                        if (a.sweeps)
-                         for (int r = 0; r < CL; ++r) cluster.map_shared_rank(s_dc, r)[k * D + dd] = x;
+                         for (int r = 0; r < CL; ++r) put(s_dc, k * D + dd, x, xbar(X_DC), r);
                      });
     }
   }
-  cluster.sync();
   if (!a.sweeps) return;
 
   const int lane = tid & 31, warp = tid >> 5;
@@ -863,6 +903,7 @@
     s_rowc[3 * a.chunk + i] = a.cov[(size_t)b * Lt + t0 + i];
   }
   __syncthreads();
+  tc::mbar_wait(xbar(X_DC), 0);
   float s1 = 0.f, s2 = 0.f;
   auto sweep7 = [&](const float* __restrict__ ea0, const float* __restrict__ ei0, auto nj_tag) {
     constexpr int NJ = decltype(nj_tag)::value;
@@ -926,16 +967,15 @@
     }
     s2 = block_sum(s2, s_red);
     if (tid < CL) {
-      float* dst = cluster.map_shared_rank(s_ex, tid) + R * 4;
-      dst[0] = s1;
-      dst[1] = s2;
-    }
-  }
-  cluster.sync();
+      put(s_ex, R * 8 + 3, s1, xbar(X_S7), tid);
+      put(s_ex, R * 8 + 4, s2, xbar(X_S7), tid);
+    }
+  }
+  tc::mbar_wait(xbar(X_S7), 0);
   float stot0 = 0.f, stot1 = 0.f;
   for (int r = 0; r < CL; ++r) {
-    stot0 += s_ex[r * 4 + 0];
-    stot1 += s_ex[r * 4 + 1];
+    stot0 += s_ex[r * 8 + 3];
+    stot1 += s_ex[r * 8 + 4];
   }
   DEC_STAMP(25);
   for (int i = tid; i < n; i += NT) {
@@ -1035,7 +1075,7 @@
     for (int q = 0; q < 2; ++q) {
       const int i = tid + q * NT;
       if (i < 3 * D)
-        for (int r = 0; r < CL; ++r) cluster.map_shared_rank(s_colp, r)[(R * 2 + m) * 3 * D + i] = xacc[q];
+        for (int r = 0; r < CL; ++r) put(s_colp, (R * 2 + m) * 3 * D + i, xacc[q], xbar(X_COLP), r);
     }
   };
   if (staged && n > 0) tc::mbar_wait(bar_proj, 0);
@@ -1050,11 +1090,10 @@
   }
   for (int i = tid; i < n; i += NT) a.d_cov[(size_t)b * Lt + t0 + i] = s_row[i];
   if (tid < CL) {
-    float* dst = cluster.map_shared_rank(s_ex, tid) + R * 4;
-    dst[2] = se_m0;
-    dst[3] = se_m1;
-  }
-  cluster.sync();
+    put(s_ex, R * 8 + 5, se_m0, xbar(X_COLP), tid);
+    put(s_ex, R * 8 + 6, se_m1, xbar(X_COLP), tid);
+  }
+  tc::mbar_wait(xbar(X_COLP), 0);
   DEC_STAMP(26);
   for (int i = tid; i < 2 * D; i += NT) {
     const int m = i / D, d = i - m * D;
@@ -1078,7 +1117,7 @@
   for (int i = tid; i < 4 * H; i += NT) s_in[i] = s_dg[i];
   if (R == 0 && tid < 2) {
     float sv = 0.f;
-    for (int r = 0; r < CL; ++r) sv += s_ex[r * 4 + 2 + tid];
+    for (int r = 0; r < CL; ++r) sv += s_ex[r * 8 + 5 + tid];
     a.scal_acc[b * 4 + tid] += sv;
   }
   __syncthreads();
@@ -1093,10 +1132,14 @@
 
 static size_t g_head_smem_set = 0;
 
+static int decoder_cluster_size(int B) { return B <= 20 ? 8 : 4; }
+constexpr size_t kSmemPerBlock = 227 * 1024;
+constexpr size_t kStaticSmem = 128;
+
 static size_t head_smem_bytes(int D, int H, int M, int CL, int chunk = 0, bool sweeps = false, int PW = NW) {
   auto up4 = [](size_t v) { return (v + 3) & ~(size_t)3; };
   const size_t per_m = (M + CL - 1) / CL;
-  size_t floats = up4(per_m) + up4((size_t)MAXC * H) + up4(4 * H) + up4(D) + up4(2 * D) + MAXC * 4 + 32 + NT;
+  size_t floats = up4(per_m) + up4((size_t)MAXC * H) + up4(4 * H) + up4(D) + up4(2 * D) + MAXC * 8 + 32 + NT;
   if (sweeps)
     floats += up4(2 * D) + up4(2 * (size_t)chunk) + up4(4 * (size_t)chunk) + up4(6 * D) + up4((size_t)PW * 3 * D) + up4(chunk) + up4((size_t)CL * 6 * D) +
               up4(4 * H + 4 * D);
@@ -1122,7 +1165,7 @@
   MMB_REQUIRE(B > 0 && Lt > 0 && D > 0 && H > 0 && E >= 0 && M > 0, MMB_ERR_INVALID,
               "%s: B=%d Lt=%d D=%d H=%d E=%d M=%d", who, B, Lt, D, H, E, M);
   MMB_REQUIRE(D <= 256, MMB_ERR_UNSUPPORTED, "%s: D=%d > 256", who, D);
-  const int CL = (long long)B * 4 * 2 <= 160 ? 8 : 4;
+  const int CL = decoder_cluster_size(B);
   size_t smem = fused_smem_bytes(Lt, D, H, E, M, CL, &a.chunk);
   MMB_REQUIRE(smem <= 200 * 1024, MMB_ERR_UNSUPPORTED, "%s: %zu B of shared memory (Lt=%d)", who, smem, Lt);
   {
@@ -1131,7 +1174,7 @@
     const size_t stage_floats = 4 + 2 * (((size_t)a.chunk * D + 3) & ~(size_t)3);
     const bool aligned = ((reinterpret_cast<uintptr_t>(a.proj_a) | reinterpret_cast<uintptr_t>(a.proj_i) |
                            reinterpret_cast<uintptr_t>(a.enc_a) | reinterpret_cast<uintptr_t>(a.enc_i)) & 15) == 0;
-    if ((D & 3) == 0 && aligned && (base_floats + stage_floats) * 4 <= 227 * 1024 && !(stage_env && atoi(stage_env) == 0)) {
+    if ((D & 3) == 0 && aligned && (base_floats + stage_floats) * 4 + kStaticSmem <= kSmemPerBlock && !(stage_env && atoi(stage_env) == 0)) {
       a.stage_off = (int)base_floats;
       smem = (base_floats + stage_floats) * 4;
     }
@@ -1154,13 +1197,15 @@
   cfg.blockDim = dim3(NT);
   cfg.dynamicSmemBytes = smem;
   cfg.stream = static_cast<cudaStream_t>(stream);
-  cudaLaunchAttribute attr[1];
+  cudaLaunchAttribute attr[2];
   attr[0].id = cudaLaunchAttributeClusterDimension;
   attr[0].val.clusterDim.x = (unsigned)CL;
   attr[0].val.clusterDim.y = 1;
   attr[0].val.clusterDim.z = 1;
+  attr[1].id = cudaLaunchAttributeProgrammaticStreamSerialization;
+  attr[1].val.programmaticStreamSerializationAllowed = 1;
   cfg.attrs = attr;
-  cfg.numAttrs = 1;
+  cfg.numAttrs = 2;
   if (g) {
     MMB_CUDA(cudaLaunchKernelEx(&cfg, dec_greedy_fused_kernel, a, *g));
     return check_launch("dec_greedy_fused_kernel");
@@ -1229,7 +1274,7 @@
   MMB_REQUIRE((!target || g_nll) && (!g_cov || (att && cov_out)), MMB_ERR_INVALID, "mmb_decoder_bwd_head: loss-term pointers");
   MMB_REQUIRE(B > 0 && Lt > 0 && D > 0 && H > 0 && M > 0 && ldd >= M && ldg >= 4 * H && H <= NT, MMB_ERR_INVALID,
               "mmb_decoder_bwd_head: B=%d Lt=%d D=%d H=%d M=%d ldd=%d ldg=%d", B, Lt, D, H, M, ldd, ldg);
-  const int CL = (long long)B * 4 * 2 <= 160 ? 8 : 4;
+  const int CL = decoder_cluster_size(B);
   HeadArgs a{probs, d_probs, target, g_nll, g_cov, out_w, gates, cell_in, cell_out, d_h_out, d_cell_out, Wcat_ctx, d_att_cov, d_cov_out,
              alpha, beta, ctx12, pb, hw, vb1, vb2, att, cov_out, Wb13, d_logits, d_gates, d_cell, datt, dcov_tot, d_pre_b, d_ctx12,
              vec_acc, scal_acc, B, Lt, D, H, M, ldd, ldg, (Lt + CL - 1) / CL,
@@ -1245,13 +1290,15 @@
   cfg.blockDim = dim3(NT);
   cfg.dynamicSmemBytes = smem;
   cfg.stream = static_cast<cudaStream_t>(stream);
-  cudaLaunchAttribute attr[1];
+  cudaLaunchAttribute attr[2];
   attr[0].id = cudaLaunchAttributeClusterDimension;
   attr[0].val.clusterDim.x = (unsigned)CL;
   attr[0].val.clusterDim.y = 1;
   attr[0].val.clusterDim.z = 1;
+  attr[1].id = cudaLaunchAttributeProgrammaticStreamSerialization;
+  attr[1].val.programmaticStreamSerializationAllowed = 1;
   cfg.attrs = attr;
-  cfg.numAttrs = 1;
+  cfg.numAttrs = 2;
   MMB_CUDA(cudaLaunchKernelEx(&cfg, dec_bwd_head_kernel, a));
   return check_launch("dec_bwd_head_kernel");
 }
@@ -1275,7 +1322,7 @@
   MMB_REQUIRE((!target || g_nll) && (!g_cov || (att && cov_out)), MMB_ERR_INVALID, "mmb_decoder_step_fused_bwd: loss-term pointers");
   MMB_REQUIRE(B > 0 && Lt > 0 && D > 0 && D <= 256 && H > 0 && M > 0 && ldd >= M && ldg >= 4 * H + 4 * D && H <= NT, MMB_ERR_INVALID,
               "mmb_decoder_step_fused_bwd: B=%d Lt=%d D=%d H=%d M=%d ldd=%d ldg=%d", B, Lt, D, H, M, ldd, ldg);
-  const int CL = (long long)B * 4 * 2 <= 160 ? 8 : 4;
+  const int CL = decoder_cluster_size(B);
   const int chunk = (Lt + CL - 1) / CL;
   HeadArgs a{probs, d_probs, target, g_nll, g_cov, out_w, gates, cell_in, cell_out, d_h_out, d_cell_out, Wcat_ctx, d_att_cov, d_cov_out,
              alpha, beta, ctx12, pb, hw, vb1, vb2, att, cov_out, Wb13, d_logits, d_gates, d_cell, datt, dcov_tot, d_pre_b, d_ctx12,
@@ -1290,7 +1337,7 @@
     const bool aligned = ((reinterpret_cast<uintptr_t>(proj_a) | reinterpret_cast<uintptr_t>(proj_i) | reinterpret_cast<uintptr_t>(enc_a) |
                            reinterpret_cast<uintptr_t>(enc_i) | reinterpret_cast<uintptr_t>(d_proj_a) |
                            reinterpret_cast<uintptr_t>(d_proj_i)) & 15) == 0;
-    if ((D & 3) == 0 && aligned && (base_floats + stage_floats) * 4 + 64 <= 227 * 1024 && !(stage_env && atoi(stage_env) == 0)) {
+    if ((D & 3) == 0 && aligned && (base_floats + stage_floats) * 4 + 64 + kStaticSmem <= kSmemPerBlock && !(stage_env && atoi(stage_env) == 0)) {
       a.stage_off = (int)base_floats;
       smem = (base_floats + stage_floats) * 4 + 64;
     }
@@ -1304,13 +1351,15 @@
   cfg.blockDim = dim3(NT);
   cfg.dynamicSmemBytes = smem;
   cfg.stream = static_cast<cudaStream_t>(stream);
-  cudaLaunchAttribute attr[1];
+  cudaLaunchAttribute attr[2];
   attr[0].id = cudaLaunchAttributeClusterDimension;
   attr[0].val.clusterDim.x = (unsigned)CL;
   attr[0].val.clusterDim.y = 1;
   attr[0].val.clusterDim.z = 1;
+  attr[1].id = cudaLaunchAttributeProgrammaticStreamSerialization;
+  attr[1].val.programmaticStreamSerializationAllowed = 1;
   cfg.attrs = attr;
-  cfg.numAttrs = 1;
+  cfg.numAttrs = 2;
   MMB_CUDA(cudaLaunchKernelEx(&cfg, dec_bwd_head_kernel, a));
   return check_launch("dec_bwd_head_kernel (whole step)");
 }
diff --git a/mmbidaf_b200/csrc/tc_common.cuh b/mmbidaf_b200/csrc/tc_common.cuh
--- a/mmbidaf_b200/csrc/tc_common.cuh
+++ b/mmbidaf_b200/csrc/tc_common.cuh
@@ -86,6 +86,31 @@
   __trap();
 }
 __device__ __forceinline__ void fence_barrier_init() { asm volatile("fence.mbarrier_init.release.cluster;" ::: "memory"); }
+
+__device__ __forceinline__ uint32_t cluster_rank() {
+  uint32_t r;
+  asm volatile("mov.u32 %0, %%cluster_ctarank;" : "=r"(r));
+  return r;
+}
+__device__ __forceinline__ uint32_t cluster_size() {
+  uint32_t n;
+  asm volatile("mov.u32 %0, %%cluster_nctarank;" : "=r"(n));
+  return n;
+}
+__device__ __forceinline__ void grid_dependency_wait() { asm volatile("griddepcontrol.wait;" ::: "memory"); }
+__device__ __forceinline__ void launch_dependents() { asm volatile("griddepcontrol.launch_dependents;" ::: "memory"); }
+__device__ __forceinline__ void cluster_arrive_relaxed() { asm volatile("barrier.cluster.arrive.relaxed.aligned;" ::: "memory"); }
+__device__ __forceinline__ void cluster_wait() { asm volatile("barrier.cluster.wait.aligned;" ::: "memory"); }
+__device__ __forceinline__ uint32_t mapa(uint32_t smem_addr, uint32_t rank) {
+  uint32_t r;
+  asm volatile("mapa.shared::cluster.u32 %0, %1, %2;" : "=r"(r) : "r"(smem_addr), "r"(rank));
+  return r;
+}
+__device__ __forceinline__ void st_async_f32(uint32_t cluster_addr, float v, uint32_t cluster_bar) {
+  asm volatile("st.async.shared::cluster.mbarrier::complete_tx::bytes.b32 [%0], %1, [%2];" ::"r"(cluster_addr), "r"(__float_as_uint(v)),
+               "r"(cluster_bar)
+               : "memory");
+}
 __device__ __forceinline__ void tc_fence_before() { asm volatile("tcgen05.fence::before_thread_sync;" ::: "memory"); }
 __device__ __forceinline__ void tc_fence_after() { asm volatile("tcgen05.fence::after_thread_sync;" ::: "memory"); }
 
```

Result: faster. 7683 (median of 6 runs) (+1.9%).
